# arnavdantuluri/StableTriton

Hardware: AMD Instinct MI355X
Metric: denoise it/s, SDXL UNet 1024x1024 50-step, bs=1 per GPU (higher is better)
Workload: dtype bf16; 1 GPU; SDXL-base UNet, latent 128x128 (1024x1024 px), bs=1/GPU, 50-step Euler-discrete loop, hipGraph mode=step, no CFG; parallelism=prompt-parallel x1, weights=synthetic seed 0, weight_broadcasts=0

## Files before the change

### stabletriton_amd/csrc/conv_thin.h

```cpp
#pragma once
#include "gemm_args.h"

template <typename T, int KMAX>
__global__ __launch_bounds__(256) void conv_thin_kernel(const GemmArgs p, int R, int chunk) {
    extern __shared__ __attribute__((aligned(16))) float wsm[];
    const T* x = (const T*)p.A;
    const T* w = (const T*)p.W;
    const int K = p.K, N = p.N;
    const int n_lo = blockIdx.y * chunk, n_hi = min(N, n_lo + chunk);
    for (int i = threadIdx.x; i < K * (n_hi - n_lo); i += 256) {
        const int nl = i / K, k = i - nl * K;
        wsm[k * chunk + nl] = Elem<T>::to_f(w[(size_t)(n_lo + nl) * K + k]);
    }
    __syncthreads();
    const int m = blockIdx.x * 256 + threadIdx.x;
    const bool live = m < p.M;
    const int mm = live ? m : 0;
    const int hw = p.Hout * p.Wout;
    const int img = mm / hw, rem = mm - img * hw;
    const int oy = rem / p.Wout, ox = rem - oy * p.Wout;
    float xin[KMAX];
#pragma unroll
    for (int k = 0; k < KMAX; ++k) xin[k] = 0.f;
    if (R == 3 && p.S == 3 && p.Cin == 4 && KMAX >= 36) {
#pragma unroll
        for (int r = 0; r < 3; ++r)
#pragma unroll
            for (int s_ = 0; s_ < 3; ++s_) {
                int iy = oy * p.stride - p.pad + r, ix = ox * p.stride - p.pad + s_;
                const int He = p.ups ? 2 * p.Hin : p.Hin, We = p.ups ? 2 * p.Win : p.Win;
                const bool ok = iy >= 0 && ix >= 0 && iy < He && ix < We;
                if (p.ups) { iy >>= 1; ix >>= 1; }
                const T* xp = x + (((size_t)img * p.Hin + (ok ? iy : 0)) * p.Win + (ok ? ix : 0)) * 4;
                float f[4];
                Out4<T>::load(xp, f);
#pragma unroll
                for (int c = 0; c < 4; ++c) xin[(r * 3 + s_) * 4 + c] = ok ? f[c] : 0.f;
            }
    } else {
        int k = 0;
        for (int r = 0; r < R; ++r)
            for (int s_ = 0; s_ < p.S; ++s_) {
                int iy = oy * p.stride - p.pad + r, ix = ox * p.stride - p.pad + s_;
                const int He = p.ups ? 2 * p.Hin : p.Hin, We = p.ups ? 2 * p.Win : p.Win;
                const bool ok = iy >= 0 && ix >= 0 && iy < He && ix < We;
                if (p.ups) { iy >>= 1; ix >>= 1; }
                const T* xp = x + (((size_t)img * p.Hin + (ok ? iy : 0)) * p.Win + (ok ? ix : 0)) * p.Cin;
                for (int c = 0; c < p.Cin; ++c, ++k) {
                    const float v = ok ? Elem<T>::to_f(xp[c]) : 0.f;
#pragma unroll
                    for (int kk = 0; kk < KMAX; ++kk) if (kk == k) xin[kk] = v;
                }
            }
    }
    for (int n0 = n_lo; n0 < n_hi; n0 += 16) {
        float acc[16];
#pragma unroll
        for (int e = 0; e < 16; ++e) acc[e] = 0.f;
#pragma unroll
        for (int k = 0; k < KMAX; ++k) {
            if (k < K) {
                const float xv = xin[k];
                const float* wr = wsm + k * chunk + (n0 - n_lo);
#pragma unroll
                for (int e = 0; e < 16; e += 4) {
                    const f32x4 w4 = *reinterpret_cast<const f32x4*>(wr + e);
                    acc[e] += xv * w4[0]; acc[e + 1] += xv * w4[1]; acc[e + 2] += xv * w4[2]; acc[e + 3] += xv * w4[3];
                }
            }
        }
        if (!live) continue;
#pragma unroll
        for (int e0 = 0; e0 < 16; e0 += 4) {
            const int co = n0 + e0;
            if (co >= N) break;
            float v[4] = {acc[e0], acc[e0 + 1], acc[e0 + 2], acc[e0 + 3]};
            if (p.epi & ST_EPI_BIAS)
                for (int e = 0; e < 4; ++e) v[e] += Elem<T>::to_f(((const T*)p.bias)[co + e]);
            if (p.epi & ST_EPI_SILU)
                for (int e = 0; e < 4; ++e) v[e] = silu_f(v[e]);
            if (p.epi & ST_EPI_ROWBIAS)
                for (int e = 0; e < 4; ++e) v[e] += Elem<T>::to_f(((const T*)p.rowbias)[(size_t)(m / p.rows_per_batch) * N + co + e]);
            if (p.epi & ST_EPI_RESIDUAL)
                for (int e = 0; e < 4; ++e) v[e] += Elem<T>::to_f(((const T*)p.residual)[(size_t)m * p.ldr + co + e]);
            Out4<T>::store((T*)p.C + (size_t)m * p.ldc + co, v);
        }
    }
}

template <typename T>
static int conv_thin_launch(const GemmArgs& a, int R, hipStream_t st) {
    const int bx = cdiv(a.M, 256);
    int ny = cdiv(1024, bx);
    if (ny > a.N / 16) ny = a.N / 16;
    if (ny < 1) ny = 1;
    const int chunk = cdiv(cdiv(a.N, ny), 16) * 16;
    ny = cdiv(a.N, chunk);
    const size_t lds = (size_t)a.K * chunk * sizeof(float);
    ST_REQUIRE(lds <= 64 * 1024, "conv2d(thin): weights do not fit LDS");
    hipLaunchKernelGGL((conv_thin_kernel<T, 64>), dim3(bx, ny), dim3(256), lds, st, a, R, chunk);
    return st_check_launch("conv2d(thin)");
}
```

### stabletriton_amd/csrc/dispatch.h

```cpp
#pragma once
#include "gemm_reg.h"
#include "gemm_dma.h"
#include "gemm8p.h"
#ifdef ST_DEV_CONFIGS
#include "../../tools/dev_kernels/gemm4w.h"
void gemm4w_bf16(const GemmArgs& a, hipStream_t st);
void gemm4w_f16(const GemmArgs& a, hipStream_t st);
void gemm4w_fp8(const GemmArgs& a, hipStream_t st);
template <typename T> static inline void gemm4w_call(const GemmArgs& a, hipStream_t st) {
    if constexpr (std::is_same<T, bf16>::value) gemm4w_bf16(a, st);
    else if constexpr (std::is_same<T, f16>::value) gemm4w_f16(a, st);
    else gemm4w_fp8(a, st);
}
#endif

static inline bool colstats_ok(const GemmArgs& a, int bm, bool lnf) {
    const bool ok = a.col_stats && !lnf && (a.N & 3) == 0 && a.rows_per_batch > 0 && a.rows_per_batch % bm == 0 &&
                    cdiv(a.M, bm) <= a.col_tiles_cap;
    if (a.col_rows_out) *a.col_rows_out = ok ? bm : 0;
    return ok;
}

template <typename T, int BM, int BN, int WGM, int WGN, int STAGES, int U, bool CONV, bool GEGLU, bool LNF, bool XA = false>
static void launch_dma_one(const GemmArgs& a, hipStream_t st, int tiles_n) {
    const size_t lds = (size_t)STAGES * U * (BM + BN) * 128 + (size_t)BM * 8 + 1024;
    const int sk = a.splitk > 1 ? a.splitk : 1;
    auto kfn = gemm_dma_kernel<T, BM, BN, WGM, WGN, STAGES, U, CONV, GEGLU, LNF, XA>;
    const bool emit_cols = colstats_ok(a, BM, LNF);
    static unsigned long long lds_ok = 0;
    ensure_dynamic_lds(kfn, lds, &lds_ok);
    GemmArgs b = a;
    {
        static const int force_pm = dev_env_int("ST_GEMM_PANELS", 0);
        const int tiles_m = cdiv(a.M, BM);
        const double abytes = CONV ? (double)a.M * a.Cin * (a.ups ? 0.25 : 1.0) * a.stride * a.stride : (double)a.M * a.K;
        const double wbytes = (double)(GEGLU ? 2 : 1) * a.N * a.K;
        int best_p = 1;
        double best = 1e300;
        for (int pm = 1; pm <= 8; pm *= 2) {
            if (pm > tiles_m) break;
            const double c = abytes * (8.0 / pm) + wbytes * pm;
            if (c < best) { best = c; best_p = pm; }
        }
        if (force_pm > 0) best_p = force_pm > tiles_m ? tiles_m : force_pm;
        b.panel_h = cdiv(tiles_m, best_p);
    }
    const int main_blocks = cdiv(a.M, BM) * tiles_n * sk;
    b.splitk = sk;
    fill_tile_map(b, cdiv(a.M, BM), tiles_n, a.K / ((128 / (int)sizeof(T)) * U));
    static const bool no_helpers = dev_env_int("ST_NO_HELPER_BLOCKS", 0) != 0;
    b.helper_blocks = (b.next_w && main_blocks <= 208 && !no_helpers) ? (256 - main_blocks > 96 ? 96 : 256 - main_blocks) : 0;
    if (!emit_cols) b.col_stats = nullptr;
    fill_next_per(b, main_blocks + b.helper_blocks);
    hipLaunchKernelGGL(kfn, dim3(main_blocks + b.helper_blocks), dim3(WGM * WGN * 64), lds, st, b);
}

template <typename T, int BM, int BN, int WGM, int WGN, int STAGES, int U, bool CONV>
static void launch_dma(const GemmArgs& a, hipStream_t st) {
    if constexpr (!CONV) {
        const bool geglu = a.epi & ST_EPI_GEGLU;
        constexpr bool PAIRS = (BN % 32 == 0);
        if (a.ln_c) {
            if constexpr (PAIRS) {
                if (geglu) { launch_dma_one<T, BM, BN, WGM, WGN, STAGES, U, false, true, true>(a, st, cdiv(a.N, BN / 2)); return; }
            }
            launch_dma_one<T, BM, BN, WGM, WGN, STAGES, U, false, false, true>(a, st, cdiv(a.N, BN));
            return;
        }
        if constexpr (PAIRS) {
            if (geglu) { launch_dma_one<T, BM, BN, WGM, WGN, STAGES, U, false, true, false>(a, st, cdiv(a.N, BN / 2)); return; }
        }
    }
    launch_dma_one<T, BM, BN, WGM, WGN, STAGES, U, CONV, false, false>(a, st, cdiv(a.N, BN));
}

enum { CFG_64x64_S4 = 0, CFG_64x64_S8 = 1, CFG_64x64_S4_U2 = 2, CFG_128x64_S4 = 3, CFG_128x64_S3_U2 = 4,
       CFG_128x128_S3 = 5, CFG_64x64_S3 = 6, CFG_64x64_W8 = 7, CFG_128x64_W8 = 8, CFG_128x128_W8 = 9,
       CFG_64x128_W8 = 10, CFG_64x128_W8_S6 = 11, CFG_128x64_W8_S6 = 12, CFG_128x128_W8_S4 = 13, CFG_64x64_W8_S8 = 14, CFG_64x128_W8_U2 = 15, CFG_128x64_W8_U2 = 16, CFG_64x64_W8_U2 = 17, CFG_256x256_W8 = 18, CFG_256x128_W8 = 19, CFG_128x128_W8_S2 = 20, CFG_128x64_W8_S3 = 21, CFG_64x128_W8_S3 = 22, CFG_128x320_W8 = 23, CFG_128x256_W8 = 24, CFG_64x320_W8 = 25, CFG_64x80_W4 = 26, CFG_128x80_W8 = 27, CFG_128x160_W8 = 28, CFG_128x128_N4_S2 = 29, CFG_128x64_N4_S3 = 30, CFG_64x128_N4_S3 = 31, CFG_256x160_W8_S2 = 32, CFG_COUNT, CFG_256x256_8P = 100, CFG_256x160_8P = 101, CFG_256x256_4W = 102 };

static inline int cfg_bn(int cfg) {
    switch (cfg) {
        case CFG_64x64_S4: case CFG_64x64_S8: case CFG_64x64_S4_U2: case CFG_128x64_S4: case CFG_128x64_S3_U2: case CFG_64x64_S3:
        case CFG_64x64_W8: case CFG_128x64_W8: case CFG_128x64_W8_S6: case CFG_64x64_W8_S8: case CFG_128x64_W8_U2:
        case CFG_64x64_W8_U2: case CFG_128x64_W8_S3: case CFG_128x64_N4_S3: return 64;
        case CFG_256x256_W8: case CFG_128x256_W8: return 256;
        case CFG_128x320_W8: case CFG_64x320_W8: return 320;
        case CFG_64x80_W4: case CFG_128x80_W8: return 80;
        case CFG_128x160_W8: case CFG_256x160_W8_S2: return 160;
        default: return 128;
    }
}

#ifdef ST_DEV_CONFIGS
extern int g_dbg_cfg, g_dbg_fusek;
#endif
static inline int forced_cfg() {
    static int v = dev_env_int("ST_GEMM_FORCE", -1);
#ifdef ST_DEV_CONFIGS
    if (g_dbg_cfg >= 0) return g_dbg_cfg;
#endif
    return v;
}

#ifndef ST_TW_128x128
#define ST_TW_128x128 1.0
#endif
#ifndef ST_TW_64x128
#define ST_TW_64x128 1.0
#endif
#ifndef ST_TW_128x64
#define ST_TW_128x64 1.0
#endif
#ifndef ST_TW_64x64
#define ST_TW_64x64 1.0
#endif
#ifndef ST_TW_128x80
#define ST_TW_128x80 1.0
#endif
#ifndef ST_TW_128x160
#define ST_TW_128x160 1.0
#endif
#ifndef ST_TW_SPLITK
#define ST_TW_SPLITK 1.0
#endif
#ifndef ST_TW_8P
#define ST_TW_8P 1.1
#endif
static inline double model_tweak(int cfg) {
    switch (cfg) {
        case 9: return ST_TW_128x128;
        case 10: return ST_TW_64x128;
        case 8: return ST_TW_128x64;
        case 7: return ST_TW_64x64;
        case 27: return ST_TW_128x80;
        case 28: return ST_TW_128x160;
        default: return 1.0;
    }
}
#ifndef ST_SPLIT_DENSE_TRIP
#define ST_SPLIT_DENSE_TRIP 1.0
#endif
#ifndef ST_SPLIT_160_TRIP
#define ST_SPLIT_160_TRIP 0.8
#endif
template <typename T, bool CONV>
static int gemm_dispatch(const GemmArgs& a_in, hipStream_t st, int depth = 0) {
    GemmArgs a = a_in;
    if (a.Ng == 0) a.Ng = a.N;
    const long n_eff = (a.epi & ST_EPI_GEGLU) ? 2L * a.N : a.N;
    auto tiles = [&](int bm, int bn) { return (long)cdiv(a.M, bm) * cdiv(n_eff, bn); };
    constexpr int KB = 128 / (int)sizeof(T);
    const char* who = CONV ? "conv2d" : "linear";
    if constexpr (frag2<T>()) {
        if (a.K % KB != 0) return st_fail("%s: fp8 / split fp32 operands need K to be a multiple of %d", who, KB);
    } else if (a.K % KB != 0) {
        if (a.stats_chunks_out) *a.stats_chunks_out = 0;
        if (tiles(128, 128) >= 240) launch_cfg<T, 128, 128, 2, 2, CONV>(a, st);
        else if (tiles(128, 64) >= 200) launch_cfg<T, 128, 64, 2, 2, CONV>(a, st);
        else launch_cfg<T, 64, 64, 2, 2, CONV>(a, st);
        return st_check_launch(who);
    }
    if constexpr (std::is_same<T, float>::value) {
        GemmArgs b = a;
        b.stats_chunks = cdiv(a.N, 64);
        if (a.stats_chunks_out) *a.stats_chunks_out = a.row_stats ? b.stats_chunks : 0;
        launch_dma<T, 64, 64, 2, 2, 4, 1, CONV>(b, st);
        return st_check_launch(who);
    } else {
        const bool even2 = (a.K % (2 * KB) == 0);
        struct Cand { int cfg, bm, bn; double trip_us; };
        static const Cand cands[] = {{CFG_128x128_W8, 128, 128, 0.53}, {CFG_64x128_W8, 64, 128, 0.34}, {CFG_128x64_W8, 128, 64, 0.32},
                                     {CFG_64x64_W8, 64, 64, 0.19}, {CFG_128x320_W8, 128, 320, 1.9}, {CFG_64x320_W8, 64, 320, 1.1},
                                     {CFG_256x128_W8, 256, 128, 0.72}, {CFG_128x80_W8, 128, 80, 0.37}, {CFG_128x160_W8, 128, 160, 0.66}};
        static const int sks[] = {1, 2, 3, 4, 6, 8};
        static const int force_sk = dev_env_int("ST_GEMM_SPLITK", -1);
        const int nk = a.K / KB;
        const long ncols = (a.epi & ST_EPI_GEGLU) ? 2L * a.N : a.N;
        const bool can_split = a.partial && !a.ln_c && force_sk != 0 && force_sk != 1;
        int cfg = CFG_64x64_W8, sk = 1;
        double best = 1e30;
        auto small_model = [&](long ncols_, int* cfg_out, int* sk_out) {
            auto tiles_ = [&](int bm, int bn) { return (long)cdiv(a.M, bm) * cdiv(ncols_, bn); };
            double best_ = 1e30;
            for (const Cand& c : cands) {
                if (frag2<T>() && c.bn == 320) continue;
                if (is_split<T>() && c.cfg == CFG_256x128_W8) continue;
                if ((a.epi & ST_EPI_GEGLU) && c.bn % 32 != 0) continue;
                const long nt = tiles_(c.bm, c.bn);
                const double trip = (is_split<T>() && c.cfg == CFG_128x160_W8 ? ST_SPLIT_160_TRIP : c.trip_us * (is_split<T>() && !CONV ? ST_SPLIT_DENSE_TRIP : 1.0)) * (CONV ? 1.6 : 1.0) * ((!CONV && sizeof(T) == 2) ? model_tweak(c.cfg) : 1.0);
                for (int k_ : sks) {
                    if (k_ > 1 && (!can_split || nk / k_ < 4 || nt > 16384)) break;
                    const double slab_mb = (double)k_ * nt * c.bm * c.bn * 4.0 / 1e6;
                    if (k_ > 1 && slab_mb * 1e6 + 65536 > (double)a.partial_bytes) break;
                    const double rounds = (double)((nt * k_ + 255) / 256);
                    const double in_round = (double)(nt * k_ < 256 ? nt * k_ : 256);
                    const double trip_bw = in_round * (c.bm + c.bn) * 128.0 / 14.0e6;
                    const double cost = rounds * (cdiv(nk, k_) * (trip > trip_bw ? trip : trip_bw) + 3.0) * (rounds > 1.0 ? 1.3 : 1.0) + (k_ > 1 ? (2.1 + 0.4 * slab_mb) * ((!CONV && sizeof(T) == 2) ? ST_TW_SPLITK : 1.0) : 0.0);
                    if (cost < best_) { best_ = cost; if (cfg_out) *cfg_out = c.cfg; if (sk_out) *sk_out = k_; }
                }
            }
            return best_;
        };
        best = small_model(ncols, &cfg, &sk);
        if constexpr (!CONV && sizeof(T) <= 2) {
            const int f = forced_cfg();
            double c256 = 1e30, c160 = 1e30;
            if (gemm8p_applies(a, 256, KB)) c256 = (double)((tiles(256, 256) + 255) / 256) * (nk * 1.65 + 4.0);
            if (gemm8p_applies(a, 160, KB)) c160 = (double)((tiles(256, 160) + 255) / 256) * (nk * 1.52 + 4.0);
#ifdef ST_DEV_CONFIGS
            if (f == CFG_256x256_4W && gemm4w_applies(a, KB)) { gemm4w_call<T>(a, st); return st_check_launch(who); }
#endif
            static const bool no_colsplit = dev_env_int("ST_NO_COLSPLIT", 0) != 0;
            if (f < 0 && depth == 0 && !no_colsplit && c256 < 1e29 && !a.row_stats && !a.col_stats && !a.q8_out && !a.sp_out && !a.row_scale) {
                const long tm = a.M / 256, total = tiles(256, 256);
                const long rem = total % 256;
                if (total > 256 && rem > 0 && rem <= 128 && 256 % tm == 0) {
                    const long full_cols = (total / 256) * (256 / tm);
                    const long rem_rows = n_eff - full_cols * 256;
                    const double c_full = (double)(total / 256) * (nk * 1.65 + 4.0);
                    const double c_split = c_full + small_model(rem_rows, nullptr, nullptr) + 2.5;
                    const double c_whole = c256 < c160 ? c256 : c160;
                    if (c_split < 0.93 * (c_whole < best ? c_whole : best)) {
                        const int bno = (a.epi & ST_EPI_GEGLU) ? 128 : 256;
                        const long n1 = full_cols * bno;
                        typedef typename OutT<T>::type TO_;
                        GemmArgs a1 = a, a2 = a;
                        a1.N = (int)n1;
                        a1.next_w = (const char*)a.W + (size_t)n1 * a.K * sizeof(T); a1.next_bytes = (size_t)(a.N - n1) * a.K * sizeof(T); a1.next_row_lines = 0; a1.next_lead_shift = 0;
                        a2.N = a.N - (int)n1;
                        a2.W = (const char*)a.W + (size_t)n1 * a.K * sizeof(T);
                        a2.C = (char*)a.C + (size_t)n1 * sizeof(TO_);
                        if (a.bias) a2.bias = (const char*)a.bias + (size_t)n1 * sizeof(TO_);
                        if (a.residual) a2.residual = (const char*)a.residual + (size_t)n1 * sizeof(TO_);
                        if (a.ln_c) { a2.ln_c = a.ln_c + n1; a2.ln_d = a.ln_d + n1; }
                        if (a.col_scale) a2.col_scale = a.col_scale + n1;
                        if (a.stats_chunks_out) *a.stats_chunks_out = 0;
                        gemm8p_launch<T, 256, 2, 4>(a1, st);
                        if (int e = st_check_launch(who)) return e;
                        return gemm_dispatch<T, CONV>(a2, st, depth + 1);
                    }
                }
            }
            const bool take256 = f == CFG_256x256_8P || (f < 0 && c256 <= c160 && c256 < ST_TW_8P * best);
            const bool take160 = f == CFG_256x160_8P || (f < 0 && c160 < c256 && c160 < ST_TW_8P * best);
            if (take256 && c256 < 1e29) { gemm8p_launch<T, 256, 2, 4>(a, st); return st_check_launch(who); }
            if (take160 && c160 < 1e29) { gemm8p_launch<T, 160, 4, 2>(a, st); return st_check_launch(who); }
        }
        if constexpr (!CONV && is_split<T>()) {
            const int f = forced_cfg();
            double c160 = 1e30;
            if (gemm8p_applies(a, 160, KB)) c160 = (double)((tiles(256, 160) + 255) / 256) * (nk * 1.15 + 5.0);
            if (c160 < 1e29 && (f == CFG_256x160_8P || (f < 0 && c160 < 0.9 * best))) { gemm8p_launch<T, 160, 4, 2>(a, st); return st_check_launch(who); }
        }
        GemmArgs b = a;
#ifdef ST_DEV_CONFIGS
        {
            static const int small_cfg = dev_env_int("ST_GEMM_SMALL_CFG", -1);
            if (small_cfg >= 0 && small_cfg < CFG_COUNT && tiles(128, 128) < 150 && sk == 1) cfg = small_cfg;
        }
#endif
        {
            static const int env_fk = dev_env_int("ST_GEMM_FUSEK", -1);
            int force_fk = env_fk;
#ifdef ST_DEV_CONFIGS
            if (g_dbg_cfg >= 0) force_fk = g_dbg_fusek;
#endif
            const int f = forced_cfg();
            if (f >= 0 && f < CFG_COUNT) {
                const bool u2 = (f == CFG_64x64_S4_U2 || f == CFG_128x64_S3_U2 || f == CFG_64x128_W8_U2 || f == CFG_128x64_W8_U2 ||
                                 f == CFG_64x64_W8_U2);
                if (!u2 || even2) { cfg = f; sk = (force_fk > 1 && can_split) ? (force_fk > nk ? nk : force_fk) : 1; }
            }
        }
        if (sk > 1) {
            int bm = 128;
            if (cfg == CFG_64x64_W8 || cfg == CFG_64x128_W8 || cfg == CFG_64x320_W8 || cfg == CFG_64x80_W4) bm = 64;
            if (cfg == CFG_256x128_W8 || cfg == CFG_256x160_W8_S2) bm = 256;
            const long nt = tiles(bm, cfg_bn(cfg));
            if (nt <= 16384 && (size_t)sk * nt * bm * cfg_bn(cfg) * 4 + 65536 <= a.partial_bytes) {
                b.splitk = sk; b.tile_counters = (int*)a.partial; b.partial = a.partial + 16384;
            }
        }
        b.stats_chunks = cdiv(a.N, cfg_bn(cfg));
        if (a.row_stats && b.stats_chunks > a.stats_capacity) return st_fail("%s: row_stats buffer holds %d chunks, %d needed", who, a.stats_capacity, b.stats_chunks);
        if (a.stats_chunks_out) *a.stats_chunks_out = a.row_stats ? b.stats_chunks : 0;
        switch (cfg) {
            case CFG_64x64_W8: launch_dma<T, 64, 64, 4, 2, 4, 1, CONV>(b, st); break;
            case CFG_128x64_W8: launch_dma<T, 128, 64, 4, 2, 4, 1, CONV>(b, st); break;
            case CFG_64x128_W8: launch_dma<T, 64, 128, 2, 4, 4, 1, CONV>(b, st); break;
            case CFG_256x128_W8: launch_dma<T, 256, 128, 4, 2, 3, 1, CONV>(b, st); break;
            case CFG_128x320_W8: launch_dma<T, 128, 320, 4, 2, 2, 1, CONV>(b, st); break;
            case CFG_64x320_W8: launch_dma<T, 64, 320, 2, 4, 3, 1, CONV>(b, st); break;
            case CFG_128x80_W8: launch_dma<T, 128, 80, 8, 1, 4, 1, CONV>(b, st); break;
            case CFG_128x160_W8:
                if constexpr (is_split<T>()) launch_dma<T, 128, 160, 4, 2, 4, 1, CONV>(b, st);
                else launch_dma<T, 128, 160, 8, 1, 4, 1, CONV>(b, st);
                break;
#ifdef ST_DEV_CONFIGS
            case CFG_64x80_W4: launch_dma<T, 64, 80, 4, 1, 6, 1, CONV>(b, st); break;
            case CFG_128x256_W8: launch_dma<T, 128, 256, 4, 2, 3, 1, CONV>(b, st); break;
            case CFG_64x64_S4: launch_dma<T, 64, 64, 2, 2, 4, 1, CONV>(b, st); break;
            case CFG_64x64_S8: launch_dma<T, 64, 64, 2, 2, 8, 1, CONV>(b, st); break;
            case CFG_64x64_S4_U2: launch_dma<T, 64, 64, 2, 2, 4, 2, CONV>(b, st); break;
            case CFG_128x64_S4: launch_dma<T, 128, 64, 2, 2, 4, 1, CONV>(b, st); break;
            case CFG_128x64_S3_U2: launch_dma<T, 128, 64, 2, 2, 3, 2, CONV>(b, st); break;
            case CFG_128x128_S3: launch_dma<T, 128, 128, 2, 2, 3, 1, CONV>(b, st); break;
            case CFG_64x64_S3: launch_dma<T, 64, 64, 2, 2, 3, 1, CONV>(b, st); break;
            case CFG_128x128_N4_S2: launch_dma<T, 128, 128, 2, 2, 2, 1, CONV>(b, st); break;
            case CFG_128x64_N4_S3: launch_dma<T, 128, 64, 2, 2, 3, 1, CONV>(b, st); break;
            case CFG_64x128_N4_S3: launch_dma<T, 64, 128, 2, 2, 3, 1, CONV>(b, st); break;
            case CFG_256x160_W8_S2: launch_dma<T, 256, 160, 4, 2, 2, 1, CONV>(b, st); break;
            case CFG_64x128_W8_S6: launch_dma<T, 64, 128, 2, 4, 6, 1, CONV>(b, st); break;
            case CFG_128x64_W8_S6: launch_dma<T, 128, 64, 4, 2, 6, 1, CONV>(b, st); break;
            case CFG_128x128_W8_S4: launch_dma<T, 128, 128, 2, 4, 3, 1, CONV>(b, st); break;
            case CFG_64x64_W8_S8: launch_dma<T, 64, 64, 4, 2, 8, 1, CONV>(b, st); break;
            case CFG_64x128_W8_U2: launch_dma<T, 64, 128, 2, 4, 3, 2, CONV>(b, st); break;
            case CFG_128x64_W8_U2: launch_dma<T, 128, 64, 4, 2, 3, 2, CONV>(b, st); break;
            case CFG_64x64_W8_U2: launch_dma<T, 64, 64, 4, 2, 4, 2, CONV>(b, st); break;
            case CFG_256x256_W8: launch_dma<T, 256, 256, 2, 4, 2, 1, CONV>(b, st); break;
            case CFG_128x128_W8_S2: launch_dma<T, 128, 128, 2, 4, 2, 1, CONV>(b, st); break;
            case CFG_128x64_W8_S3: launch_dma<T, 128, 64, 4, 2, 3, 1, CONV>(b, st); break;
            case CFG_64x128_W8_S3: launch_dma<T, 64, 128, 2, 4, 3, 1, CONV>(b, st); break;
#endif
            default: launch_dma<T, 128, 128, 2, 4, 4, 1, CONV>(b, st); break;
        }
        return st_check_launch(who);
    }
}


static inline void take_hint(GemmArgs& a, const void* next_w, size_t next_bytes) {
    const size_t row_lines = (next_bytes >> 40) & 0xfffff, shift = (next_bytes >> 60) & 3;
    next_bytes &= ((size_t)1 << 40) - 1;
    a.next_row_lines = 0; a.next_lead_shift = 0;
    if (next_w && row_lines && (row_lines >> shift) >= 2 && next_bytes >= (row_lines << 7)) {
        const size_t rows = (next_bytes >> 7) / row_lines;
        a.next_row_lines = (unsigned)row_lines; a.next_lead_shift = (unsigned)shift;
        next_bytes = (rows << shift) << 7;
    }
    a.next_w = next_bytes ? next_w : nullptr;
    a.next_bytes = next_w ? next_bytes : 0;
}

static inline int check_epilogue(const char* who, const GemmArgs& a) {
    ST_REQUIRE(!(a.epi & ST_EPI_BIAS) || a.bias, "%s: ST_EPI_BIAS without bias pointer", who);
    ST_REQUIRE(!(a.epi & ST_EPI_RESIDUAL) || a.residual, "%s: ST_EPI_RESIDUAL without residual pointer", who);
    ST_REQUIRE(!(a.epi & ST_EPI_ROWBIAS) || (a.rowbias && a.rows_per_batch > 0), "%s: ST_EPI_ROWBIAS needs rowbias and rows_per_batch", who);
    ST_REQUIRE(!((a.epi & ST_EPI_GEGLU) && (a.epi & ST_EPI_SILU)), "%s: GEGLU and SILU are exclusive", who);
    return 0;
}
```

### stabletriton_amd/csrc/gemm8p.h

```cpp
#pragma once
#include "gemm_dma.h"

template <int BN, int WGM, int WGN> constexpr bool TILE_OK_SPLIT() { return (256 / WGM / 16) * (BN / WGN / 16) <= 20; }
template <typename T, bool GEGLU, bool LNF, int BN = 256, int WGM = 2, int WGN = 4, bool DIRECT = false>
__global__ __launch_bounds__(512) void gemm8p_kernel(const GemmArgs p) {
    static_assert(sizeof(T) <= 2 || is_split<T>(), "16-bit elements (bf16 / f16), e4m3 bytes, or split fp32 operands (strict mode: 256 x 160 tiles)");
    static_assert(!is_split<T>() || (TILE_OK_SPLIT<BN, WGM, WGN>()), "split operands carry two accumulator sets: wave tiles of at most 64 x 80");
    constexpr int BM = 256, NW = 8;
    constexpr int KB = 128 / (int)sizeof(T);
    constexpr int EV = 16 / (int)sizeof(T);
    typedef typename OutT<T>::type TO;
    static_assert(WGM * WGN == NW && BM % (32 * WGM) == 0 && BN % (16 * WGN) == 0 && (!GEGLU || BN % 32 == 0), "wave layout");
    constexpr int WTM = BM / WGM, WTN = BN / WGN, TM = WTM / 16, TN = WTN / 16;
    constexpr int TMH = TM / 2, TN0 = (TN + 1) / 2, TN1 = TN - TN0;
    constexpr int RA = WGM * TMH * 16, RB0 = WGN * TN0 * 16, RB1 = WGN * TN1 * 16;
    static_assert(RA == 128 && RB0 <= 128 && RB1 <= 128 && RB0 % 8 == 0 && RB1 % 8 == 0, "a region is at most sixteen 8-row pieces");
    constexpr int HA = RA * 128, HB0 = RB0 * 128, HB1 = RB1 * 128;
    constexpr int TILE_B = 2 * HA + HB0 + HB1;
    constexpr int BNO = GEGLU ? BN / 2 : BN;
    typedef typename Mma<T>::Frag Frag;
    typedef typename std::conditional<frag2<T>(), u32x4, Frag>::type Half;
    extern __shared__ __attribute__((aligned(16))) char lds[];
    char* const lnrows = lds + 2 * TILE_B;
    char* const dump = lnrows + BM * 8;

    const int t = threadIdx.x, lane = t & 63;
    const int wave = __builtin_amdgcn_readfirstlane(t >> 6);
    const int wm = wave / WGN, wn = wave - wm * WGN;
    const int tiles_m = p.M / BM;
    const int nblk = gridDim.x - p.helper_blocks, bid = blockIdx.x;
    if (bid >= nblk) {
        unsigned int sink = 0;
        touch_next_weights(p, sink, true);
        retire_touches(sink);
        return;
    }
    const TileId tid = tile_of_block(p, bid, nblk);
    const int tile_m = tid.tile_m, tile_n = tid.tile_n;
    const int m0 = tile_m * BM, n0 = tile_n * BNO;
#ifdef ST_PROBE8
    unsigned long long pr_t0 = __builtin_readcyclecounter(), pr_t1 = 0, pr_t2 = 0, pr_r0 = __builtin_amdgcn_s_memrealtime();
#endif
    const T* __restrict__ Ap = (const T*)p.A;
    const T* __restrict__ Wp = (const T*)p.W;
    const T* zeros = reinterpret_cast<const T*>(g_zero16);

    const int lr = lane >> 3;
    const int lc = (lane & 7) ^ lr;
    const T* a_src[2];
    const T* b0_src[2];
    const T* b1_src[2];
    auto w_row = [&](int c) { return GEGLU ? (c < BN / 2 ? (size_t)(n0 + c) : (size_t)p.Ng + n0 + (c - BN / 2)) : (size_t)(n0 + c); };
    auto w_row_direct = [&](int wc, int j, int rho) {
        const DirectCol dc = direct_col<TN, GEGLU>(j, rho);
        return (size_t)(dc.gate ? p.Ng : 0) + n0 + wc * (GEGLU ? WTN / 2 : WTN) + dc.col;
    };
#pragma unroll
    for (int e = 0; e < 2; ++e) {
        const int idx = (2 * wave + e) * 8 + lr;
        a_src[e] = Ap + (size_t)(m0 + (idx / (TMH * 16)) * WTM + (idx % (TMH * 16))) * p.lda + lc * EV;
        const int i0 = idx < RB0 ? idx : 0, i1 = idx < RB1 ? idx : 0;
        if constexpr (DIRECT) {
            const int in0 = i0 % (TN0 * 16), in1 = i1 % (TN1 * 16);
            b0_src[e] = Wp + w_row_direct(i0 / (TN0 * 16), in0 >> 4, in0 & 15) * p.K + lc * EV;
            b1_src[e] = Wp + w_row_direct(i1 / (TN1 * 16), TN0 + (in1 >> 4), in1 & 15) * p.K + lc * EV;
        } else {
            b0_src[e] = Wp + w_row((i0 / (TN0 * 16)) * WTN + (i0 % (TN0 * 16))) * p.K + lc * EV;
            b1_src[e] = Wp + w_row((i1 / (TN1 * 16)) * WTN + TN0 * 16 + (i1 % (TN1 * 16))) * p.K + lc * EV;
        }
    }
    const size_t a_half = (size_t)(TMH * 16) * p.lda;
    const int nk = p.K / KB;

    auto issue_half = [&](int kt, int region) {
#ifdef ST_PROBE8
        if (p.korder & 2) kt = nk;
#endif
        const int roff = region == 0 ? 0 : region == 1 ? HA : region == 2 ? 2 * HA : 2 * HA + HB0;
        const int rrows = region < 2 ? RA : region == 2 ? RB0 : RB1;
        const unsigned dst = lds_addr_of(lds) + (kt & 1) * TILE_B + roff + (2 * wave) * 1024;
#pragma unroll
        for (int e = 0; e < 2; ++e) {
            const bool live = kt < nk && (2 * wave + e) * 8 < rrows;
            const T* src = region < 2 ? a_src[e] + (region & 1) * a_half : region == 2 ? b0_src[e] : b1_src[e];
            src = live ? src + (size_t)kt * KB : zeros;
            dma16_at<0>(src, live ? dst + e * 1024 : lds_addr_of(lds) + 2 * TILE_B + BM * 8);
        }
    };

    unsigned int touch_sink = 0;
    {
        auto touch_at = [&](const char* a) {
            a = (const char*)((uintptr_t)a & ~(uintptr_t)3);
            asm volatile("global_load_dword %0, %1, off" : "+v"(touch_sink) : "v"(a) : "memory");
        };
        auto touch = [&](const void* base, long byte_off, int nbytes) {
            for (int o = t * 128; o < nbytes; o += 512 * 128) touch_at((const char*)base + byte_off + o);
        };
        if (p.epi & ST_EPI_BIAS) {
            touch(p.bias, (long)n0 * (long)sizeof(TO), BNO * (int)sizeof(TO));
            if (GEGLU) touch(p.bias, ((long)p.Ng + n0) * (long)sizeof(TO), BNO * (int)sizeof(TO));
        }
        if (LNF) {
            touch(p.ln_c, (long)n0 * 4, BNO * 4); touch(p.ln_d, (long)n0 * 4, BNO * 4);
            if (GEGLU) { touch(p.ln_c, ((long)p.Ng + n0) * 4, BNO * 4); touch(p.ln_d, ((long)p.Ng + n0) * 4, BNO * 4); }
        }
        if (p.epi & ST_EPI_RESIDUAL) {
            constexpr int lines = (BNO * (int)sizeof(TO) + 127) / 128;
            for (int o = t; o < BM * lines; o += 512) {
                const int r = o / lines, l = o - r * lines;
                touch_at((const char*)p.residual + ((size_t)(m0 + r) * p.ldr + n0) * sizeof(TO) + l * 128);
            }
        }
    }
    LnRowSum<2> ln_sum;
    if constexpr (LNF) {
        const float2* st2 = reinterpret_cast<const float2*>(p.ln_stats);
        const int row = t >> 1, part = t & 1;
        ln_sum.load(st2 + (size_t)(m0 + row) * p.ln_chunks, p.ln_chunks, part);
    }
    issue_half(0, 0); issue_half(0, 2); issue_half(0, 3); issue_half(0, 1); issue_half(1, 0); issue_half(1, 2); issue_half(1, 3);
    if constexpr (LNF) {
        const float2* st2 = reinterpret_cast<const float2*>(p.ln_stats);
        const int row = t >> 1, part = t & 1;
        float a1, a2;
        ln_sum.finish(st2 + (size_t)(m0 + row) * p.ln_chunks, p.ln_chunks, part, a1, a2);
        const float mean = a1 / (float)p.K;
        const float rstd = rsqrtf(fmaxf(a2 / (float)p.K - mean * mean, 0.f) + p.ln_eps);
        if (part == 0) reinterpret_cast<float2*>(lnrows)[row] = make_float2(mean, rstd);
        asm volatile("s_waitcnt lgkmcnt(0)" ::: "memory");
    }
    wait_vmcnt<8>();
    __builtin_amdgcn_s_barrier();
    asm volatile("" ::"v"(touch_sink));
    if (wave >= 4) __builtin_amdgcn_s_barrier();

    f32x4 acc[TM][TN];
    f32x4 corr[is_split<T>() ? TM : 1][is_split<T>() ? TN : 1];
#pragma unroll
    for (int i = 0; i < TM; ++i)
#pragma unroll
        for (int j = 0; j < TN; ++j) {
            acc[i][j] = (f32x4){0.f, 0.f, 0.f, 0.f};
            if constexpr (is_split<T>()) corr[i][j] = (f32x4){0.f, 0.f, 0.f, 0.f};
        }

    const int r16 = lane & 15, q = lane >> 4;
    int a_off[2], b0_off[2], b1_off[2];
#pragma unroll
    for (int kk = 0; kk < 2; ++kk) {
        const int sw = ((4 * kk + q) ^ (r16 & 7)) << 4;
        a_off[kk] = (wm * TMH * 16 + r16) * 128 + sw;
        b0_off[kk] = 2 * HA + (wn * TN0 * 16 + r16) * 128 + sw;
        b1_off[kk] = 2 * HA + HB0 + (wn * TN1 * 16 + r16) * 128 + sw;
    }
    constexpr int NKK = frag2<T>() ? 1 : 2;
    Frag fa[TMH][NKK], fb[TN][NKK];
    auto read_op = [&](const char* base, const int (&off)[2], Frag (&dst)[NKK]) {
        if constexpr (frag2<T>()) {
            const Half lo = *reinterpret_cast<const Half*>(base + off[0]), hi = *reinterpret_cast<const Half*>(base + off[1]);
            dst[0] = Frag{(int)lo[0], (int)lo[1], (int)lo[2], (int)lo[3], (int)hi[0], (int)hi[1], (int)hi[2], (int)hi[3]};
        } else {
#pragma unroll
            for (int kk = 0; kk < 2; ++kk) dst[kk] = *reinterpret_cast<const Frag*>(base + off[kk]);
        }
    };
    auto read_a = [&](const char* tile, int h) {
#pragma unroll
        for (int i = 0; i < TMH; ++i) read_op(tile + h * HA + i * 2048, a_off, fa[i]);
    };
    auto read_b = [&](const char* tile) {
#pragma unroll
        for (int j = 0; j < TN0; ++j) read_op(tile + j * 2048, b0_off, fb[j]);
#pragma unroll
        for (int j = 0; j < TN1; ++j) read_op(tile + j * 2048, b1_off, fb[TN0 + j]);
    };
    auto half_tile = [&](auto mh_) {
        constexpr int mh = decltype(mh_)::value;
#ifdef ST_PROBE8
        if (p.korder & 1) return;
#endif
        __builtin_amdgcn_s_setprio(1);
#pragma unroll
        for (int kk = 0; kk < NKK; ++kk)
#pragma unroll
            for (int i = 0; i < TMH; ++i)
#pragma unroll
                for (int j = 0; j < TN; ++j) {
                    if constexpr (is_split<T>()) Mma<T>::run2(acc[mh * TMH + i][j], corr[mh * TMH + i][j], fb[j][kk], fa[i][kk]);
                    else Mma<T>::run(acc[mh * TMH + i][j], fb[j][kk], fa[i][kk]);
                }
        __builtin_amdgcn_s_setprio(0);
    };
#define ST_PHASE_SYNC()                                   \
    __builtin_amdgcn_sched_barrier(0);                    \
    wait_vmcnt<8>();                                      \
    __builtin_amdgcn_s_barrier();                         \
    __builtin_amdgcn_sched_barrier(0)
#define ST_PHASE_END()                                    \
    __builtin_amdgcn_sched_barrier(0);                    \
    __builtin_amdgcn_s_barrier();                         \
    __builtin_amdgcn_sched_barrier(0)
    typedef std::integral_constant<int, 0> I0;
    typedef std::integral_constant<int, 1> I1;
#ifdef ST_PROBE8
    pr_t1 = __builtin_readcyclecounter();
#endif
    for (int kt = 0; kt < nk; ++kt) {
        const char* tile = lds + (kt & 1) * TILE_B;
        read_a(tile, 0); read_b(tile);
        issue_half(kt + 1, 1);
        ST_PHASE_SYNC();
        half_tile(I0{});
        ST_PHASE_END();
        read_a(tile, 1);
        issue_half(kt + 2, 0); issue_half(kt + 2, 2); issue_half(kt + 2, 3);
        ST_PHASE_SYNC();
        half_tile(I1{});
        ST_PHASE_END();
    }
#undef ST_PHASE_SYNC
#undef ST_PHASE_END
    if (wave < 4) __builtin_amdgcn_s_barrier();
    wait_vmcnt<0>();
    __builtin_amdgcn_s_barrier();
#ifdef ST_PROBE8
    pr_t2 = __builtin_readcyclecounter();
#endif
    if constexpr (is_split<T>()) {
#pragma unroll
        for (int i = 0; i < TM; ++i)
#pragma unroll
            for (int j = 0; j < TN; ++j)
#pragma unroll
                for (int e = 0; e < 4; ++e) acc[i][j][e] = __builtin_fmaf(corr[i][j][e], ST_SPLIT_INV, acc[i][j][e]);
    }
    if constexpr (DIRECT)
        direct_epilogue<TO, TM, TN, WTM, WTN, WGM, WGN, GEGLU, LNF>(p, acc, m0, n0, tile_n, wm, wn, r16, q, lds, reinterpret_cast<const float2*>(lnrows),
                                                                    lds_addr_of(lds) + 2 * TILE_B + BM * 8);
    else
        staged_epilogue<TO, BM, BN, WGM, WGN, TM, TN, GEGLU, 2 * TILE_B, !LNF, is_fp8<T>()>(p, acc, m0, n0, tile_n, wm, r16, q, ColsPlain{wn, WTN}, lds,
                                                                            reinterpret_cast<const float2*>(lnrows));
#ifdef ST_PROBE8
    asm volatile("s_waitcnt vmcnt(0)" ::: "memory");
    if (p.partial && t == 0) {
        unsigned long long* o = reinterpret_cast<unsigned long long*>(reinterpret_cast<char*>(p.partial) + 65536) + (size_t)bid * 8;
        o[0] = pr_t0; o[1] = pr_t1; o[2] = pr_t2; o[3] = __builtin_readcyclecounter(); o[4] = pr_r0; o[5] = __builtin_amdgcn_s_memrealtime();
    }
#endif
}

static inline bool gemm8p_applies(const GemmArgs& a, int bn, int kb = 64) {
    const long n_rows = (a.epi & ST_EPI_GEGLU) ? 2L * a.N : a.N;
    return a.M % 256 == 0 && n_rows % bn == 0 && a.K % kb == 0 && a.K >= 2 * kb && a.N % 8 == 0 &&
           !(a.epi & ST_EPI_ROWBIAS) && (!a.row_stats || !(a.epi & ST_EPI_GEGLU));
}

template <typename T, bool GEGLU, bool LNF, int BN, int WGM, int WGN, bool DIRECT = false>
static void gemm8p_go(const GemmArgs& a, hipStream_t st) {
    constexpr size_t lds = 2 * (size_t)(2 * 128 * 128 + BN * 128) + 256 * 8 + 1024;
    auto kfn = gemm8p_kernel<T, GEGLU, LNF, BN, WGM, WGN, DIRECT>;
    static unsigned long long lds_ok = 0;
    ensure_dynamic_lds(kfn, lds, &lds_ok);
    GemmArgs b = a;
    const int tiles_m = a.M / 256, tiles_n = (int)(((a.epi & ST_EPI_GEGLU) ? 2L * a.N : a.N) / BN);
    {
        const double abytes = (double)a.M * a.K, wbytes = (double)tiles_n * BN * a.K;
        int best_p = 1;
        double best = 1e300;
        for (int pm = 1; pm <= 8 && pm <= tiles_m; pm *= 2) {
            const double c = abytes * (8.0 / pm) + wbytes * pm;
            if (c < best) { best = c; best_p = pm; }
        }
        b.panel_h = cdiv(tiles_m, best_p);
    }
    const int main_blocks = tiles_m * tiles_n;
    b.splitk = 1;
    fill_tile_map(b, tiles_m, tiles_n, 0);
    b.helper_blocks = (b.next_w && main_blocks <= 208) ? (256 - main_blocks > 96 ? 96 : 256 - main_blocks) : 0;
    b.stats_chunks = tiles_n;
    if (a.stats_chunks_out) *a.stats_chunks_out = a.row_stats ? b.stats_chunks : 0;
    if (!colstats_ok(a, 256, LNF)) b.col_stats = nullptr;
    fill_next_per(b, main_blocks + b.helper_blocks);
    hipLaunchKernelGGL(kfn, dim3(main_blocks + b.helper_blocks), dim3(512), lds, st, b);
}

template <typename T>
static inline bool gemm8p_direct(const GemmArgs& a, bool tall) {
    if constexpr (sizeof(T) != 2) return false;
    static const bool off = dev_env_int("ST_8P_STAGED", 0) != 0;
    if (off || direct_flags(a, a.ln_c != nullptr, tall) < 0) return false;
    auto al16 = [](const void* p_) { return ((uintptr_t)p_ & 15) == 0; };
    return a.ldc % 8 == 0 && al16(a.C) && (!(a.epi & ST_EPI_RESIDUAL) || (a.ldr % 8 == 0 && al16(a.residual))) && al16(a.bias) && al16(a.ln_c) && al16(a.ln_d);
}

template <typename T, int BN, int WGM, int WGN>
static void gemm8p_launch(const GemmArgs& a, hipStream_t st) {
    const bool geglu = a.epi & ST_EPI_GEGLU;
    if constexpr (sizeof(T) == 2) {
        if (gemm8p_direct<T>(a, 256 / WGM / 16 >= 8)) {
            if (a.ln_c) { if (geglu) gemm8p_go<T, true, true, BN, WGM, WGN, true>(a, st); else gemm8p_go<T, false, true, BN, WGM, WGN, true>(a, st); }
            else { if (geglu) gemm8p_go<T, true, false, BN, WGM, WGN, true>(a, st); else gemm8p_go<T, false, false, BN, WGM, WGN, true>(a, st); }
            return;
        }
    }
    if (a.ln_c) { if (geglu) gemm8p_go<T, true, true, BN, WGM, WGN>(a, st); else gemm8p_go<T, false, true, BN, WGM, WGN>(a, st); }
    else { if (geglu) gemm8p_go<T, true, false, BN, WGM, WGN>(a, st); else gemm8p_go<T, false, false, BN, WGM, WGN>(a, st); }
}
```

### stabletriton_amd/csrc/gemm_api.hip

```cpp
#include "gemm_core.h"

#ifdef ST_DEV_CONFIGS
int g_dbg_cfg = -1, g_dbg_fusek = -1;
extern "C" void st_debug_force_gemm(int cfg, int fusek) { g_dbg_cfg = cfg; g_dbg_fusek = fusek; }
#endif

static int run_dense(const GemmArgs& a, int dtype, hipStream_t st) {
    switch (dtype) {
        case ST_BF16: return gemm_dense_bf16(a, st);
        case ST_F16: return gemm_dense_f16(a, st);
        case ST_F32S: return gemm_dense_f32s(a, st);
        default: return gemm_dense_f32(a, st);
    }
}

static int check_q8(const char* who, GemmArgs& a, void* q8, long ldq8, const float* q8_inv_scale, unsigned int* q8_amax) {
    if (!q8) return 0;
    ST_REQUIRE(q8_inv_scale && q8_amax, "%s: the e4m3 copy needs its scale and its amax slots", who);
    ST_REQUIRE(a.N % 8 == 0 && ldq8 % 8 == 0 && (uintptr_t)q8 % 8 == 0, "%s: e4m3 copy: N and its row stride must be multiples of 8", who);
    a.q8_out = q8; a.q8_ld = ldq8; a.q8_inv_scale = q8_inv_scale; a.q8_amax = q8_amax;
    return 0;
}

static int linear_impl(const void* x, const void* W, const void* bias, const void* residual, const void* rowbias, void* y,
                       int M, int N, int K, long lda, long ldc, long ldr, int rows_per_batch, int epilogue, int dtype,
                       void* workspace, size_t workspace_bytes, float* row_stats, int row_stats_capacity,
                       int* row_stats_chunks, float* col_stats, int col_stats_tiles, int* col_stats_rows,
                       void* q8, long ldq8, const float* q8_inv_scale, unsigned int* q8_amax,
                       const void* next_weights, size_t next_weights_bytes, void* stream) {
    if (col_stats_rows) *col_stats_rows = 0;
    ST_REQUIRE(x && W && y, "linear: null pointer");
    ST_REQUIRE(M > 0 && N > 0 && K > 0, "linear: bad shape M=%d N=%d K=%d", M, N, K);
    ST_REQUIRE(st_dtype_ok_gemm(dtype), "linear: unsupported dtype %d", dtype);
    const int vec = st_dtype_is16(dtype) ? 8 : (dtype == ST_F32S ? 32 : 4);
    ST_REQUIRE(K % vec == 0 && lda % vec == 0, "linear: K=%d and lda=%ld must be multiples of %d", K, lda, vec);
    ST_REQUIRE(ldc % 4 == 0 && (!(epilogue & ST_EPI_RESIDUAL) || ldr % 4 == 0), "linear: ldc/ldr must be multiples of 4");
    ST_REQUIRE(((uintptr_t)x | (uintptr_t)W) % 16 == 0 && (uintptr_t)y % 16 == 0, "linear: pointers must be 16-byte aligned");
    GemmArgs a = {};
    a.A = x; a.W = W; a.bias = bias; a.residual = residual; a.rowbias = rowbias; a.C = y;
    a.M = M; a.N = N; a.K = K; a.lda = lda; a.ldc = ldc; a.ldr = ldr; a.rows_per_batch = rows_per_batch; a.epi = epilogue;
    a.splitk = 1; a.partial = (float*)workspace; a.partial_bytes = workspace ? workspace_bytes : 0;
    ST_REQUIRE(!row_stats || !(epilogue & ST_EPI_GEGLU), "linear: row_stats with GEGLU is not supported");
    a.row_stats = row_stats; a.stats_capacity = row_stats_capacity; a.stats_chunks_out = row_stats_chunks;
    a.col_stats = col_stats; a.col_tiles_cap = col_stats_tiles; a.col_rows_out = col_stats_rows;
    take_hint(a, next_weights, next_weights_bytes);
#ifdef ST_PROBE8
    { const char* e_ = getenv("ST_PROBE_KNOB"); a.korder = e_ ? atoi(e_) : 0; }
#endif
    if (int e = check_epilogue("linear", a)) return e;
    if (q8) {
        ST_REQUIRE(st_dtype_is16(dtype), "linear: the e4m3 copy is emitted by the 16-bit kernels");
        if (int e = check_q8("linear", a, q8, ldq8, q8_inv_scale, q8_amax)) return e;
    }
    if (int e = st_take_split_arm("linear", M, N, !st_dtype_is16(dtype) && N % 32 == 0, &a.sp_out)) return e;
    return run_dense(a, dtype, (hipStream_t)stream);
}

extern "C" int st_linear(const void* x, const void* W, const void* bias, const void* residual, const void* rowbias, void* y,
                         int M, int N, int K, long lda, long ldc, long ldr, int rows_per_batch, int epilogue, int dtype,
                         void* workspace, size_t workspace_bytes, float* row_stats, int row_stats_capacity,
                         int* row_stats_chunks, float* col_stats, int col_stats_tiles, int* col_stats_rows,
                         const void* next_weights, size_t next_weights_bytes, void* stream) {
    return linear_impl(x, W, bias, residual, rowbias, y, M, N, K, lda, ldc, ldr, rows_per_batch, epilogue, dtype, workspace, workspace_bytes,
                       row_stats, row_stats_capacity, row_stats_chunks, col_stats, col_stats_tiles, col_stats_rows, nullptr, 0, nullptr, nullptr,
                       next_weights, next_weights_bytes, stream);
}

extern "C" int st_linear_emit8(const void* x, const void* W, const void* bias, const void* residual, const void* rowbias, void* y,
                               int M, int N, int K, long lda, long ldc, long ldr, int rows_per_batch, int epilogue, int dtype,
                               void* workspace, size_t workspace_bytes, float* row_stats, int row_stats_capacity,
                               int* row_stats_chunks, float* col_stats, int col_stats_tiles, int* col_stats_rows,
                               void* q8, long ldq8, const float* q8_inv_scale, unsigned int* q8_amax,
                               const void* next_weights, size_t next_weights_bytes, void* stream) {
    ST_REQUIRE(q8, "linear_emit8: null e4m3 output");
    return linear_impl(x, W, bias, residual, rowbias, y, M, N, K, lda, ldc, ldr, rows_per_batch, epilogue, dtype, workspace, workspace_bytes,
                       row_stats, row_stats_capacity, row_stats_chunks, col_stats, col_stats_tiles, col_stats_rows, q8, ldq8, q8_inv_scale, q8_amax,
                       next_weights, next_weights_bytes, stream);
}

extern "C" int st_ln_linear(const void* x, const float* row_stats, int row_stats_chunks, const void* Wg, const float* c,
                            const float* d, void* y, int M, int N, int K, long lda, long ldc, float eps, int epilogue,
                            int dtype, const void* next_weights, size_t next_weights_bytes, void* stream) {
    ST_REQUIRE(x && Wg && c && d && y && row_stats, "ln_linear: null pointer");
    ST_REQUIRE(row_stats_chunks > 0, "ln_linear: the producer emitted no row statistics");
    ST_REQUIRE(M > 0 && N > 0 && K > 0, "ln_linear: bad shape M=%d N=%d K=%d", M, N, K);
    ST_REQUIRE(st_dtype_ok_gemm(dtype), "ln_linear: unsupported dtype %d", dtype);
    const int kb = st_dtype_is16(dtype) ? 64 : 32;
    ST_REQUIRE(K % kb == 0 && lda % (dtype == ST_F32S ? 32 : kb / 8) == 0, "ln_linear: K=%d must be a multiple of %d", K, kb);
    ST_REQUIRE(ldc % 4 == 0, "ln_linear: ldc must be a multiple of 4");
    ST_REQUIRE((epilogue & ~ST_EPI_GEGLU) == 0, "ln_linear: only the GEGLU epilogue flag is accepted (bias lives in d)");
    ST_REQUIRE(((uintptr_t)x | (uintptr_t)Wg | (uintptr_t)y) % 16 == 0, "ln_linear: pointers must be 16-byte aligned");
    GemmArgs a = {};
    a.A = x; a.W = Wg; a.C = y; a.M = M; a.N = N; a.K = K; a.lda = lda; a.ldc = ldc; a.epi = epilogue;
    a.ln_c = c; a.ln_d = d; a.ln_eps = eps; a.splitk = 1; a.ln_stats = row_stats; a.ln_chunks = row_stats_chunks;
    take_hint(a, next_weights, next_weights_bytes);
    if (int e = st_take_split_arm("ln_linear", M, N, !st_dtype_is16(dtype) && N % 32 == 0, &a.sp_out)) return e;
    return run_dense(a, dtype, (hipStream_t)stream);
}

extern "C" int st_ln_linear_xattn(const void* x, const float* row_stats, int row_stats_chunks, const void* Wg, const float* c,
                                  const float* d, const void* k, const void* v, void* out, int M, int N, int K, long lda, long ldo,
                                  float eps, int rows_per_batch, int S, int H, long ldk, long ldv, float scale, int dtype,
                                  const void* next_weights, size_t next_weights_bytes, void* stream) {
    ST_REQUIRE(st_dtype_is16(dtype), "ln_linear_xattn: dtype %d not supported (bf16 / f16)", dtype);
    ST_REQUIRE(x && Wg && c && d && k && v && out && row_stats, "ln_linear_xattn: null pointer");
    ST_REQUIRE(row_stats_chunks > 0, "ln_linear_xattn: the producer emitted no row statistics");
    ST_REQUIRE(M > 0 && N > 0 && K > 0 && S > 0 && H > 0, "ln_linear_xattn: bad shape M=%d N=%d K=%d S=%d H=%d", M, N, K, S, H);
    ST_REQUIRE(N == H * 64, "ln_linear_xattn: N=%d must be H*64 (H=%d)", N, H);
    ST_REQUIRE(S < 256, "ln_linear_xattn: context of %d keys (the fused epilogue runs the short-context attention core: S < 256)", S);
    ST_REQUIRE(rows_per_batch > 0 && rows_per_batch % 128 == 0 && M % rows_per_batch == 0,
               "ln_linear_xattn: %d rows per batch: query tiles of 128 rows must not straddle batches", rows_per_batch);
    ST_REQUIRE(K % 64 == 0 && lda % 8 == 0 && ldo % 4 == 0 && ldk % 8 == 0 && ldv % 8 == 0, "ln_linear_xattn: K, strides must keep 16-byte alignment");
    ST_REQUIRE(((uintptr_t)x | (uintptr_t)Wg | (uintptr_t)out | (uintptr_t)k | (uintptr_t)v | (uintptr_t)c | (uintptr_t)d) % 16 == 0,
               "ln_linear_xattn: pointers must be 16-byte aligned");
    GemmArgs a = {};
    a.A = x; a.W = Wg; a.C = out; a.M = M; a.N = N; a.K = K; a.lda = lda; a.ldc = ldo; a.epi = 0;
    a.ln_c = c; a.ln_d = d; a.ln_eps = eps; a.splitk = 1; a.ln_stats = row_stats; a.ln_chunks = row_stats_chunks;
    a.xa_k = k; a.xa_v = v; a.xa_ldk = ldk; a.xa_ldv = ldv; a.xa_S = S; a.xa_T = rows_per_batch; a.xa_scale_log2e = scale * 1.4426950408889634f;
    take_hint(a, next_weights, next_weights_bytes);
    { void* none; if (int e = st_take_split_arm("ln_linear_xattn", M, N, false, &none)) return e; }
    return dtype == ST_BF16 ? gemm_xattn_bf16(a, (hipStream_t)stream) : gemm_xattn_f16(a, (hipStream_t)stream);
}

extern "C" int st_linear_fp8(const void* xq, const float* row_scale, const void* Wq, const float* w_scale, const void* bias,
                             const void* residual, void* y, int M, int N, int K, long lda, long ldc, long ldr, int epilogue,
                             void* workspace, size_t workspace_bytes, const void* next_weights, size_t next_weights_bytes,
                             void* stream) {
    ST_REQUIRE(xq && row_scale && Wq && w_scale && y, "linear_fp8: null pointer");
    ST_REQUIRE(M > 0 && N > 0 && K > 0, "linear_fp8: bad shape M=%d N=%d K=%d", M, N, K);
    ST_REQUIRE(K % 128 == 0 && lda % 16 == 0, "linear_fp8: K=%d must be a multiple of 128 and lda=%ld of 16", K, lda);
    ST_REQUIRE(N % 4 == 0 && ldc % 4 == 0 && (!(epilogue & ST_EPI_RESIDUAL) || ldr % 4 == 0), "linear_fp8: N, ldc, ldr must be multiples of 4");
    ST_REQUIRE(!(epilogue & ST_EPI_ROWBIAS), "linear_fp8: the row-bias epilogue is not supported");
    ST_REQUIRE(((uintptr_t)xq | (uintptr_t)Wq | (uintptr_t)y | (uintptr_t)w_scale) % 16 == 0, "linear_fp8: pointers must be 16-byte aligned");
    GemmArgs a = {};
    a.A = xq; a.W = Wq; a.bias = bias; a.residual = residual; a.C = y;
    a.M = M; a.N = N; a.K = K; a.lda = lda; a.ldc = ldc; a.ldr = ldr; a.epi = epilogue;
    a.row_scale = row_scale; a.col_scale = w_scale; a.rs_stride = 1;
    a.splitk = 1; a.partial = (float*)workspace; a.partial_bytes = workspace ? workspace_bytes : 0;
    take_hint(a, next_weights, next_weights_bytes);
    if (int e = check_epilogue("linear_fp8", a)) return e;
    return gemm_dense_fp8(a, (hipStream_t)stream);
}

extern "C" int st_linear_fp8x(const void* xq, const float* a_scale, int a_scale_stride, const void* Wq, const float* w_scale,
                              const void* bias, const void* residual, void* y, int M, int N, int K, long lda, long ldc, long ldr, int epilogue,
                              const float* ln_stats, int ln_chunks, const float* ln_c, const float* ln_d, float ln_eps,
                              float* row_stats, int row_stats_capacity, int* row_stats_chunks,
                              void* q8, long ldq8, const float* q8_inv_scale, unsigned int* q8_amax,
                              void* workspace, size_t workspace_bytes, const void* next_weights, size_t next_weights_bytes, void* stream) {
    ST_REQUIRE(xq && a_scale && Wq && w_scale && (y || q8), "linear_fp8x: null pointer");
    ST_REQUIRE(a_scale_stride == 0 || a_scale_stride == 1, "linear_fp8x: activation scale stride %d (0 = per tensor, 1 = per row)", a_scale_stride);
    ST_REQUIRE(M > 0 && N > 0 && K > 0, "linear_fp8x: bad shape M=%d N=%d K=%d", M, N, K);
    ST_REQUIRE(K % 128 == 0 && lda % 16 == 0, "linear_fp8x: K=%d must be a multiple of 128 and lda=%ld of 16", K, lda);
    ST_REQUIRE(N % 4 == 0 && (!y || ldc % 4 == 0) && (!(epilogue & ST_EPI_RESIDUAL) || ldr % 4 == 0), "linear_fp8x: N, ldc, ldr must be multiples of 4");
    ST_REQUIRE(!(epilogue & ST_EPI_ROWBIAS), "linear_fp8x: the row-bias epilogue is not supported");
    ST_REQUIRE(((uintptr_t)xq | (uintptr_t)Wq | (uintptr_t)y | (uintptr_t)w_scale) % 16 == 0, "linear_fp8x: pointers must be 16-byte aligned");
    ST_REQUIRE(!ln_c || (ln_d && ln_stats && ln_chunks > 0 && !(epilogue & ~ST_EPI_GEGLU)), "linear_fp8x: folded LayerNorm takes c, d, the row statistics and only the GEGLU flag (bias lives in d)");
    ST_REQUIRE(y || (epilogue & ST_EPI_GEGLU), "linear_fp8x: an output without y (only the e4m3 copy) is the GEGLU form");
    GemmArgs a = {};
    a.A = xq; a.W = Wq; a.bias = bias; a.residual = residual; a.C = y;
    a.M = M; a.N = N; a.K = K; a.lda = lda; a.ldc = ldc; a.ldr = ldr; a.epi = epilogue;
    a.row_scale = a_scale; a.col_scale = w_scale; a.rs_stride = a_scale_stride;
    a.ln_c = ln_c; a.ln_d = ln_d; a.ln_eps = ln_eps; a.ln_stats = ln_stats; a.ln_chunks = ln_chunks;
    a.splitk = 1; a.partial = (float*)workspace; a.partial_bytes = workspace ? workspace_bytes : 0;
    ST_REQUIRE(!row_stats || !(epilogue & ST_EPI_GEGLU), "linear_fp8x: row_stats with GEGLU is not supported");
    a.row_stats = row_stats; a.stats_capacity = row_stats_capacity; a.stats_chunks_out = row_stats_chunks;
    take_hint(a, next_weights, next_weights_bytes);
    if (int e = check_epilogue("linear_fp8x", a)) return e;
    if (int e = check_q8("linear_fp8x", a, q8, ldq8, q8_inv_scale, q8_amax)) return e;
    return gemm_dense_fp8(a, (hipStream_t)stream);
}

extern "C" int st_conv2d(const void* x, const void* W, const void* bias, const void* residual, const void* rowbias, void* y,
                         int N, int Hin, int Win, int Cin, int Cout, int R, int S, int stride, int pad, int upsample2x,
                         int epilogue, int dtype, void* workspace, size_t workspace_bytes,
                         float* col_stats, int col_stats_tiles, int* col_stats_rows,
                         const void* next_weights, size_t next_weights_bytes, void* stream) {
    if (col_stats_rows) *col_stats_rows = 0;
    ST_REQUIRE(x && W && y, "conv2d: null pointer");
    ST_REQUIRE(N > 0 && Hin > 0 && Win > 0 && Cin > 0 && Cout > 0 && R > 0 && S > 0 && stride > 0 && pad >= 0,
               "conv2d: bad geometry");
    ST_REQUIRE(st_dtype_ok_gemm(dtype), "conv2d: unsupported dtype %d", dtype);
    ST_REQUIRE(!(epilogue & ST_EPI_GEGLU), "conv2d: GEGLU epilogue not supported");
    ST_REQUIRE(Cout % 4 == 0, "conv2d: Cout=%d must be a multiple of 4", Cout);
    const int He = upsample2x ? 2 * Hin : Hin, We = upsample2x ? 2 * Win : Win;
    GemmArgs a = {};
    a.A = x; a.W = W; a.bias = bias; a.residual = residual; a.rowbias = rowbias; a.C = y;
    a.Hin = Hin; a.Win = Win; a.Cin = Cin; a.S = S; a.stride = stride; a.pad = pad; a.ups = upsample2x ? 1 : 0;
    {
        static const int korder_env = dev_env_int("ST_CONV_KORDER", -1);
        a.R_ = R; a.korder = korder_env >= 0 ? korder_env : 0;
    }
    a.Hout = (He + 2 * pad - R) / stride + 1;
    a.Wout = (We + 2 * pad - S) / stride + 1;
    ST_REQUIRE(a.Hout > 0 && a.Wout > 0, "conv2d: empty output");
    a.M = N * a.Hout * a.Wout; a.N = Cout; a.K = R * S * Cin;
    a.lda = 0; a.ldc = Cout; a.ldr = Cout; a.rows_per_batch = a.Hout * a.Wout; a.epi = epilogue;
    a.splitk = 1; a.partial = (float*)workspace; a.partial_bytes = workspace ? workspace_bytes : 0;
    a.col_stats = col_stats; a.col_tiles_cap = col_stats_tiles; a.col_rows_out = col_stats_rows;
    take_hint(a, next_weights, next_weights_bytes);
    if (int e = check_epilogue("conv2d", a)) return e;
    if (int e = st_take_split_arm("conv2d", a.M, Cout, !st_dtype_is16(dtype) && Cout % 32 == 0 && Cin % 32 == 0, &a.sp_out)) return e;
    hipStream_t st = (hipStream_t)stream;
    const int kb = st_dtype_is16(dtype) ? 64 : 32;
    if (Cin % kb == 0) {
        ST_REQUIRE(((uintptr_t)x | (uintptr_t)W | (uintptr_t)y) % 16 == 0, "conv2d: pointers must be 16-byte aligned");
        if (dtype == ST_BF16) return gemm_conv_bf16(a, R, upsample2x, st);
        if (dtype == ST_F16) return gemm_conv_f16(a, R, upsample2x, st);
        if (dtype == ST_F32S) return gemm_conv_f32s(a, R, upsample2x, st);
        return gemm_conv_f32(a, st);
    }
    ST_REQUIRE(dtype != ST_F32S, "conv2d: split fp32 operands need Cin=%d to be a multiple of 32 (thin inputs take plain ST_F32)", Cin);
    ST_REQUIRE(a.K <= 64 && Cout % 16 == 0, "conv2d: Cin=%d is neither a multiple of %d (implicit GEMM) nor thin (R*S*Cin <= 64, Cout %% 16 == 0)", Cin, kb);
    return conv_thin_run(a, R, dtype, st);
}

extern "C" int st_conv1x1_cat(const void* x0, int C0, const void* x1, int C1, const void* W, const void* bias, const void* residual, void* y,
                              int N, int H, int Wd, int Cout, int epilogue, int dtype, void* workspace, size_t workspace_bytes,
                              float* col_stats, int col_stats_tiles, int* col_stats_rows,
                              const void* next_weights, size_t next_weights_bytes, void* stream) {
    if (col_stats_rows) *col_stats_rows = 0;
    ST_REQUIRE(x0 && x1 && W && y, "conv1x1_cat: null pointer");
    ST_REQUIRE(N > 0 && H > 0 && Wd > 0 && C0 > 0 && C1 > 0 && Cout > 0, "conv1x1_cat: bad geometry");
    ST_REQUIRE(st_dtype_ok_gemm(dtype), "conv1x1_cat: unsupported dtype %d", dtype);
    ST_REQUIRE(!(epilogue & (ST_EPI_GEGLU | ST_EPI_ROWBIAS)), "conv1x1_cat: GEGLU / row-bias epilogues not supported");
    ST_REQUIRE(Cout % 4 == 0, "conv1x1_cat: Cout=%d must be a multiple of 4", Cout);
    const int kb = st_dtype_is16(dtype) ? 64 : 32;
    ST_REQUIRE(C0 % kb == 0 && C1 % kb == 0, "conv1x1_cat: both channel counts (%d, %d) must be multiples of %d", C0, C1, kb);
    ST_REQUIRE(((uintptr_t)x0 | (uintptr_t)x1 | (uintptr_t)W | (uintptr_t)y) % 16 == 0, "conv1x1_cat: pointers must be 16-byte aligned");
    GemmArgs a = {};
    a.A = x0; a.A2 = x1; a.Csplit = C0; a.W = W; a.bias = bias; a.residual = residual; a.C = y;
    a.Hin = H; a.Win = Wd; a.Cin = C0 + C1; a.S = 1; a.stride = 1; a.pad = 0; a.ups = 0; a.R_ = 1; a.korder = 0;
    a.Hout = H; a.Wout = Wd;
    a.M = N * H * Wd; a.N = Cout; a.K = C0 + C1;
    a.lda = 0; a.ldc = Cout; a.ldr = Cout; a.rows_per_batch = H * Wd; a.epi = epilogue;
    a.splitk = 1; a.partial = (float*)workspace; a.partial_bytes = workspace ? workspace_bytes : 0;
    a.col_stats = col_stats; a.col_tiles_cap = col_stats_tiles; a.col_rows_out = col_stats_rows;
    take_hint(a, next_weights, next_weights_bytes);
    if (int e = check_epilogue("conv1x1_cat", a)) return e;
    if (int e = st_take_split_arm("conv1x1_cat", a.M, Cout, !st_dtype_is16(dtype) && Cout % 32 == 0, &a.sp_out)) return e;
    hipStream_t st = (hipStream_t)stream;
    if (dtype == ST_BF16) return gemm_conv_bf16(a, 1, 0, st);
    if (dtype == ST_F16) return gemm_conv_f16(a, 1, 0, st);
    if (dtype == ST_F32S) return gemm_conv_f32s(a, 1, 0, st);
    return gemm_conv_f32(a, st);
}
```

### stabletriton_amd/csrc/gemm_args.h

```cpp
#pragma once
#include "common.h"
#include "attention_core.h"
#include "split.h"
#include <stdlib.h>
#include <type_traits>

struct GemmArgs {
    const void* A; const void* W; const void* bias; const void* residual; const void* rowbias; void* C;
    int M, N, K;
    int Ng;
    long lda, ldc, ldr;
    int rows_per_batch;
    int epi;
    int Hin, Win, Cin, Hout, Wout, S, stride, pad, ups;
    int R_, korder;
    const float* ln_c; const float* ln_d; float ln_eps;
    const float* ln_stats; int ln_chunks;
    float* row_stats; int stats_chunks;
    int stats_capacity; int* stats_chunks_out;
    float* col_stats; int col_tiles_cap; int* col_rows_out;
    int splitk;
    float* partial;
    size_t partial_bytes;
    int* tile_counters;
    int panel_h;
    const void* A2; int Csplit;
    int tm_tiles_m, tm_per_panel, tm_last_rows, tm_slow;
    unsigned tm_mg_splitk, tm_mg_per_panel, tm_mg_rows, tm_mg_last;
    int nk_base, nk_rem;
    unsigned next_per;
    unsigned next_row_lines;
    unsigned next_lead_shift;
    const float* row_scale; const float* col_scale;
    int rs_stride;
    void* q8_out; long q8_ld; const float* q8_inv_scale; unsigned int* q8_amax;
    void* sp_out;
    const void* next_w; size_t next_bytes;
    int helper_blocks;
    const void* xa_k; const void* xa_v; long xa_ldk, xa_ldv; int xa_S, xa_T; float xa_scale_log2e;
};

static inline int dev_env_int(const char* name, int dflt) {
#ifdef ST_DEV_CONFIGS
    const char* e = getenv(name);
    return e ? atoi(e) : dflt;
#else
    (void)name;
    return dflt;
#endif
}

static inline bool colstats_ok(const GemmArgs& a, int bm, bool lnf);

template <typename T> struct Mma;
template <> struct Mma<bf16> {
    typedef bf16x8 Frag;
    static __device__ __forceinline__ void run(f32x4& acc, const Frag& a, const Frag& b) {
        acc = __builtin_amdgcn_mfma_f32_16x16x32_bf16(a, b, acc, 0, 0, 0);
    }
};
template <> struct Mma<f16> {
    typedef f16x8 Frag;
    static __device__ __forceinline__ void run(f32x4& acc, const Frag& a, const Frag& b) {
        acc = __builtin_amdgcn_mfma_f32_16x16x32_f16(a, b, acc, 0, 0, 0);
    }
};
template <> struct Mma<float> {
    typedef f32x4 Frag;
    static __device__ __forceinline__ void run(f32x4& acc, const Frag& a, const Frag& b) {
#pragma unroll
        for (int j = 0; j < 4; ++j) acc = __builtin_amdgcn_mfma_f32_16x16x4f32(a[j], b[j], acc, 0, 0, 0);
    }
};

struct f8 { unsigned char v; };
typedef __attribute__((ext_vector_type(8))) int i32x8;
template <> struct Mma<f8> {
    typedef i32x8 Frag;
    static __device__ __forceinline__ void run(f32x4& acc, const Frag& a, const Frag& b) {
        acc = __builtin_amdgcn_mfma_scale_f32_16x16x128_f8f6f4(a, b, acc, 0 , 0 , 0, 0x7F7F7F7F, 0, 0x7F7F7F7F);
    }
};
struct fsp { float raw; };
template <> struct Mma<fsp> {
    typedef i32x8 Frag;
    static __device__ __forceinline__ void run2(f32x4& acc, f32x4& corr, const Frag& a, const Frag& b) {
        typedef __attribute__((ext_vector_type(4))) int i32x4_;
        const f16x8 ah = __builtin_bit_cast(f16x8, (i32x4_)__builtin_shufflevector(a, a, 0, 1, 2, 3));
        const f16x8 al = __builtin_bit_cast(f16x8, (i32x4_)__builtin_shufflevector(a, a, 4, 5, 6, 7));
        const f16x8 bh = __builtin_bit_cast(f16x8, (i32x4_)__builtin_shufflevector(b, b, 0, 1, 2, 3));
        const f16x8 bl = __builtin_bit_cast(f16x8, (i32x4_)__builtin_shufflevector(b, b, 4, 5, 6, 7));
        acc = __builtin_amdgcn_mfma_f32_16x16x32_f16(ah, bh, acc, 0, 0, 0);
        corr = __builtin_amdgcn_mfma_f32_16x16x32_f16(ah, bl, corr, 0, 0, 0);
        corr = __builtin_amdgcn_mfma_f32_16x16x32_f16(al, bh, corr, 0, 0, 0);
    }
};
static constexpr float ST_SPLIT_INV = 1.0f / 2048.0f;
template <typename T> constexpr bool is_fp8() { return std::is_same<T, f8>::value; }
template <typename T> constexpr bool is_split() { return std::is_same<T, fsp>::value; }
template <typename T> constexpr bool frag2() { return is_fp8<T>() || is_split<T>(); }
template <typename T> struct OutT { typedef T type; };
template <> struct OutT<f8> { typedef bf16 type; };
template <> struct OutT<fsp> { typedef float type; };
template <typename T> constexpr int mfma_per_frag() { return is_split<T>() ? 3 : (sizeof(T) == 4 ? 4 : 1); }

template <typename T> struct Out4;
template <> struct Out4<bf16> {
    static __device__ __forceinline__ void load(const bf16* p, float* f) {
        bf16x4 v = *reinterpret_cast<const bf16x4*>(p);
#pragma unroll
        for (int i = 0; i < 4; ++i) f[i] = (float)v[i];
    }
    static __device__ __forceinline__ void store(bf16* p, const float* f) {
        bf16x4 v;
#pragma unroll
        for (int i = 0; i < 4; ++i) v[i] = (bf16)f[i];
        *reinterpret_cast<bf16x4*>(p) = v;
    }
};
template <> struct Out4<f16> {
    static __device__ __forceinline__ void load(const f16* p, float* f) {
        f16x4 v = *reinterpret_cast<const f16x4*>(p);
#pragma unroll
        for (int i = 0; i < 4; ++i) f[i] = (float)v[i];
    }
    static __device__ __forceinline__ void store(f16* p, const float* f) {
        f16x4 v;
#pragma unroll
        for (int i = 0; i < 4; ++i) v[i] = (f16)f[i];
        *reinterpret_cast<f16x4*>(p) = v;
    }
};
template <> struct Out4<float> {
    static __device__ __forceinline__ void load(const float* p, float* f) {
        f32x4 v = *reinterpret_cast<const f32x4*>(p);
#pragma unroll
        for (int i = 0; i < 4; ++i) f[i] = v[i];
    }
    static __device__ __forceinline__ void store(float* p, const float* f) {
        f32x4 v = {f[0], f[1], f[2], f[3]};
        *reinterpret_cast<f32x4*>(p) = v;
    }
};


__device__ __forceinline__ size_t touch_line(const GemmArgs& p, size_t l) {
    if (!p.next_row_lines) return l;
    return (l >> p.next_lead_shift) * p.next_row_lines + (l & ((1u << p.next_lead_shift) - 1u));
}
__device__ __forceinline__ void touch_next_weights(const GemmArgs& p, unsigned int& sink, bool helper = false) {
    if (!p.next_w || (p.helper_blocks > 0) != helper) return;
    const size_t lines = p.next_bytes >> 7;
    const size_t nsl = helper ? p.helper_blocks : gridDim.x;
    const size_t me = helper ? blockIdx.x - (gridDim.x - p.helper_blocks) : blockIdx.x;
    const size_t per = p.next_per ? (size_t)p.next_per : (lines + nsl - 1) / nsl;
    const size_t lo = me * per, hi = lo + per < lines ? lo + per : lines;
    const size_t step = blockDim.x;
    for (size_t l = lo + threadIdx.x; l < hi; l += step) {
        const char* a_ = (const char*)p.next_w + (touch_line(p, l) << 7);
        asm volatile("global_load_dword %0, %1, off" : "+v"(sink) : "v"(a_) : "memory");
    }
}
__device__ __forceinline__ void retire_touches(unsigned int& sink) { asm volatile("s_waitcnt vmcnt(0)" : "+v"(sink)::"memory"); }

static inline unsigned magic_u32(unsigned d) { return d <= 1 ? 0u : (unsigned)((1ull << 32) / d + 1); }
__device__ __forceinline__ int mg_div(int n, unsigned mg) { return mg ? (int)__umulhi((unsigned)n, mg) : n; }

struct TileId { int tile_m, tile_n, split, tw; };
__device__ __forceinline__ TileId tile_of_block(const GemmArgs& p, int bid, int nblk) {
    const int xq = nblk >> 3, xr = nblk & 7, xcd = bid & 7;
    const int wg = (xcd < xr ? xcd * (xq + 1) : xr * (xq + 1) + (xcd - xr) * xq) + (bid >> 3);
    TileId r;
    if (p.tm_slow) {
        r.split = wg % p.splitk; r.tw = wg / p.splitk;
        const int pn = r.tw / p.tm_per_panel, rem = r.tw - pn * p.tm_per_panel;
        const int rows = min(p.panel_h, p.tm_tiles_m - pn * p.panel_h);
        r.tile_n = rem / rows;
        r.tile_m = pn * p.panel_h + (rem - r.tile_n * rows);
        return r;
    }
    r.tw = mg_div(wg, p.tm_mg_splitk);
    r.split = wg - r.tw * p.splitk;
    const int pn = mg_div(r.tw, p.tm_mg_per_panel), rem = r.tw - pn * p.tm_per_panel;
    const bool last = (pn + 1) * p.panel_h > p.tm_tiles_m;
    const int rows = last ? p.tm_last_rows : p.panel_h;
    r.tile_n = mg_div(rem, last ? p.tm_mg_last : p.tm_mg_rows);
    r.tile_m = pn * p.panel_h + (rem - r.tile_n * rows);
    return r;
}
static inline void fill_tile_map(GemmArgs& b, int tiles_m, int tiles_n, int nk_stages) {
    const int sk = b.splitk > 1 ? b.splitk : 1;
    b.splitk = sk;
    b.tm_tiles_m = tiles_m;
    b.tm_per_panel = b.panel_h * tiles_n;
    b.tm_last_rows = tiles_m % b.panel_h ? tiles_m % b.panel_h : b.panel_h;
    b.tm_mg_splitk = magic_u32((unsigned)sk);
    b.tm_mg_per_panel = magic_u32((unsigned)b.tm_per_panel);
    b.tm_mg_rows = magic_u32((unsigned)b.panel_h);
    b.tm_mg_last = magic_u32((unsigned)b.tm_last_rows);
    const unsigned long long blocks = (unsigned long long)tiles_m * tiles_n * sk;
    b.tm_slow = (blocks * (unsigned long long)(b.tm_per_panel > sk ? b.tm_per_panel : sk) >= (1ull << 32)) ? 1 : 0;
    b.nk_base = nk_stages / sk;
    b.nk_rem = nk_stages % sk;
}
static inline void fill_next_per(GemmArgs& b, unsigned grid) {
    const size_t lines = b.next_bytes >> 7;
    const size_t nsl = b.helper_blocks > 0 ? (size_t)b.helper_blocks : (size_t)grid;
    b.next_per = (b.next_w && nsl) ? (unsigned)((lines + nsl - 1) / nsl) : 0u;
}

template <typename T> struct Raw4;
template <> struct Raw4<bf16> { typedef bf16x4 type; };
template <> struct Raw4<f16> { typedef f16x4 type; };
template <> struct Raw4<float> { typedef f32x4 type; };
template <typename T> __device__ __forceinline__ typename Raw4<T>::type ld_raw4(const T* p) {
    return *reinterpret_cast<const typename Raw4<T>::type*>(p);
}

__device__ __forceinline__ float row16_sum(float v) {
    v += __builtin_bit_cast(float, __builtin_amdgcn_update_dpp(0, __builtin_bit_cast(int, v), 0xB1, 0xF, 0xF, false));
    v += __builtin_bit_cast(float, __builtin_amdgcn_update_dpp(0, __builtin_bit_cast(int, v), 0x4E, 0xF, 0xF, false));
    v += __builtin_bit_cast(float, __builtin_amdgcn_update_dpp(0, __builtin_bit_cast(int, v), 0x124, 0xF, 0xF, false));
    v += __builtin_bit_cast(float, __builtin_amdgcn_update_dpp(0, __builtin_bit_cast(int, v), 0x128, 0xF, 0xF, false));
    return v;
}

__device__ __forceinline__ float ln_fold(float acc, float mean, float rstd, float c, float d) {
    return __builtin_fmaf(rstd, __builtin_fmaf(-mean, c, acc), d);
}

int gemm_dense_bf16(const GemmArgs& a, hipStream_t st);
int gemm_dense_f16(const GemmArgs& a, hipStream_t st);
int gemm_dense_f32(const GemmArgs& a, hipStream_t st);
int gemm_dense_f32s(const GemmArgs& a, hipStream_t st);
int gemm_dense_fp8(const GemmArgs& a, hipStream_t st);
int gemm_xattn_bf16(const GemmArgs& a, hipStream_t st);
int gemm_xattn_f16(const GemmArgs& a, hipStream_t st);
int gemm_conv_bf16(const GemmArgs& a, int R, int ups, hipStream_t st);
int gemm_conv_f16(const GemmArgs& a, int R, int ups, hipStream_t st);
int gemm_conv_f32(const GemmArgs& a, hipStream_t st);
int gemm_conv_f32s(const GemmArgs& a, int R, int ups, hipStream_t st);
int conv_thin_run(const GemmArgs& a, int R, int dtype, hipStream_t st);
```

### stabletriton_amd/csrc/gemm_dma.h

```cpp
#pragma once
#include "epilogue.h"

static __device__ __attribute__((aligned(16))) unsigned int g_zero16[4] = {0u, 0u, 0u, 0u};

typedef __attribute__((address_space(3))) void lds_void_t;
typedef __attribute__((address_space(1))) const void gbl_cvoid_t;

template <int AUX = 0>
__device__ __forceinline__ void dma16(const void* src, char* lds_wave_base) {
    __builtin_amdgcn_global_load_lds((gbl_cvoid_t*)src, (lds_void_t*)lds_wave_base, 16, 0, AUX);
}

constexpr int dma_before_last_group(int G, int NG) {
    int n = 0;
    for (int e = 0; e < G; ++e) n += (e * NG / G < NG - 1) ? 1 : 0;
    return n;
}

constexpr int dma_in_group(int G, int NG, int g) {
    int n = 0;
    for (int e = 0; e < G; ++e) n += (e * NG / G == g) ? 1 : 0;
    return n;
}

template <int AUX = 0>
__device__ __forceinline__ void dma16_at(const void* src, unsigned lds_addr) {
    __builtin_amdgcn_global_load_lds((gbl_cvoid_t*)src, (lds_void_t*)(uintptr_t)lds_addr, 16, 0, AUX);
}
__device__ __forceinline__ unsigned lds_addr_of(const char* p) { return (unsigned)(uintptr_t)(lds_void_t*)p; }

template <int N> __device__ __forceinline__ void wait_vmcnt() {
    asm volatile("s_waitcnt vmcnt(%0)" ::"n"(N) : "memory");
}


template <int TPR>
struct LnRowSum {
    static_assert(TPR == 1 || TPR == 2 || TPR == 4 || TPR == 8, "threads per row");
    static constexpr int RES = 8 / TPR;
    static constexpr int PRE = 8 / RES;
    float2 pre[RES][PRE];
    __device__ __forceinline__ void load(const float2* row, int chunks, int part) {
#pragma unroll
        for (int j = 0; j < RES; ++j)
#pragma unroll
            for (int i = 0; i < PRE; ++i) {
                const int c = part + TPR * j + 8 * i;
                pre[j][i] = row[c < chunks ? c : 0];
            }
    }
    __device__ __forceinline__ void finish(const float2* row, int chunks, int part, float& s1, float& s2) {
        float a1[RES], a2[RES];
#pragma unroll
        for (int j = 0; j < RES; ++j) {
            a1[j] = 0.f; a2[j] = 0.f;
#pragma unroll
            for (int i = 0; i < PRE; ++i) {
                const bool ok = part + TPR * j + 8 * i < chunks;
                a1[j] += ok ? pre[j][i].x : 0.f; a2[j] += ok ? pre[j][i].y : 0.f;
            }
            for (int c = part + TPR * j + 8 * PRE; c < chunks; c += 8) { const float2 v = row[c]; a1[j] += v.x; a2[j] += v.y; }
#pragma unroll
            for (int o = 1; o < TPR; o <<= 1) { a1[j] += __shfl_xor(a1[j], o, 64); a2[j] += __shfl_xor(a2[j], o, 64); }
        }
#pragma unroll
        for (int w = 1; w < RES; w <<= 1)
#pragma unroll
            for (int j = 0; j + w < RES; j += 2 * w) { a1[j] += a1[j + w]; a2[j] += a2[j + w]; }
        s1 = a1[0]; s2 = a2[0];
    }
};

template <int TM, int TN, int TILE_ELEMS>
__device__ __forceinline__ bool splitk_combine(const GemmArgs& p, f32x4 (&acc)[TM][TN], int tw, int split, char* lds, int t, int wave, int lane) {
    float* slab0 = p.partial + (size_t)tw * p.splitk * TILE_ELEMS;
    {
        asm volatile("s_nop 7\n\ts_nop 7\n\ts_nop 2" ::: "memory");
        float* mine = slab0 + (size_t)split * TILE_ELEMS + (size_t)wave * (TM * TN * 256) + lane * 4;
#pragma unroll
        for (int i = 0; i < TM; ++i)
#pragma unroll
            for (int j = 0; j < TN; ++j) {
                const float* dst = mine + (i * TN + j) * 256;
                asm volatile("global_store_dwordx4 %0, %1, off sc1\n\ts_nop 1" ::"v"(dst), "v"(acc[i][j]) : "memory");
            }
    }
    asm volatile("s_waitcnt vmcnt(0)" ::: "memory");
    __syncthreads();
    int* flag = reinterpret_cast<int*>(lds);
    if (t == 0) *flag = __hip_atomic_fetch_add(p.tile_counters + tw, 1, __ATOMIC_RELAXED, __HIP_MEMORY_SCOPE_AGENT);
    __syncthreads();
    if (*flag != p.splitk - 1) return false;
    if (t == 0) __hip_atomic_store(p.tile_counters + tw, 0, __ATOMIC_RELAXED, __HIP_MEMORY_SCOPE_AGENT);
    f32x4 own[TM][TN];
#pragma unroll
    for (int i = 0; i < TM; ++i)
#pragma unroll
        for (int j = 0; j < TN; ++j) { own[i][j] = acc[i][j]; acc[i][j] = (f32x4){0.f, 0.f, 0.f, 0.f}; }
    typedef unsigned int u32x4_ __attribute__((ext_vector_type(4)));
    const __amdgpu_buffer_rsrc_t slabs = __builtin_amdgcn_make_buffer_rsrc((void*)slab0, 0, (int)((size_t)p.splitk * TILE_ELEMS * 4), 0x00020000);
    for (int sl = 0; sl < p.splitk; ++sl) {
        if (sl == split) {
#pragma unroll
            for (int i = 0; i < TM; ++i)
#pragma unroll
                for (int j = 0; j < TN; ++j) acc[i][j] += own[i][j];
            continue;
        }
        const int off = (sl * TILE_ELEMS + wave * (TM * TN * 256) + lane * 4) * 4;
#pragma unroll
        for (int i = 0; i < TM; ++i)
#pragma unroll
            for (int j = 0; j < TN; ++j)
                acc[i][j] += __builtin_bit_cast(f32x4, (u32x4_)__builtin_amdgcn_raw_buffer_load_b128(slabs, off + (i * TN + j) * 1024, 0, 16));
    }
    return true;
}

template <typename T, int BM, int BN, int WGM, int WGN, int STAGES, int U, bool CONV, bool GEGLU, bool LNF = false, bool XA = false>
__global__ __launch_bounds__(WGM* WGN * 64) void gemm_dma_kernel(const GemmArgs p) {
    constexpr int NW = WGM * WGN;
    constexpr int VEC = 16 / (int)sizeof(T);
    constexpr int KB = 8 * VEC;
    constexpr int WTM = BM / WGM, WTN = BN / WGN;
    constexpr int TM = WTM / 16, TN = WTN / 16;
    constexpr int A_PIECES = BM / 8, B_PIECES = BN / 8;
    constexpr int A_IT = (A_PIECES + NW - 1) / NW, B_IT = (B_PIECES + NW - 1) / NW;
    constexpr bool UNEVEN = (A_PIECES % NW != 0) || (B_PIECES % NW != 0);
    constexpr int G = (A_IT + B_IT) * U;
    constexpr int A_BYTES = BM * 128, TILE = (BM + BN) * 128, STAGE = TILE * U;
    static_assert(!GEGLU || (BN % 32 == 0), "GEGLU: value and gate halves of the tile are whole 16-column accumulator tiles");
    static_assert((STAGES - 2) * G <= 63, "vmcnt immediate");
    typedef typename Mma<T>::Frag Frag;
    typedef typename OutT<T>::type TO;

    extern __shared__ __attribute__((aligned(16))) char lds[];
    char* const dump = lds + STAGES * STAGE + BM * 8;

    const int t = threadIdx.x, lane = t & 63;
    const int wave = __builtin_amdgcn_readfirstlane(t >> 6);
    const int wm = wave / WGN, wn = wave - wm * WGN;
    const int tiles_m = (p.M + BM - 1) / BM;
    const int nblk = gridDim.x - p.helper_blocks, bid = blockIdx.x;
    if (bid >= nblk) {
        unsigned int sink = 0;
        touch_next_weights(p, sink, true);
        retire_touches(sink);
        return;
    }
    constexpr int BNO = GEGLU ? BN / 2 : BN;
    const TileId tid = tile_of_block(p, bid, nblk);
    const int split = tid.split, tw = tid.tw, tile_m = tid.tile_m, tile_n = tid.tile_n;
    const int m0 = tile_m * BM;
    const int n0 = tile_n * BNO;

    const T* __restrict__ Ap = (const T*)p.A;
    const T* __restrict__ Wp = (const T*)p.W;
    const T* zeros = reinterpret_cast<const T*>(g_zero16);

    const int lr = lane >> 3;
    const int lc = (lane & 7) ^ lr;
    const T* a_ptr[A_IT];
    const T* a2_ptr[CONV ? A_IT : 1];
    int a_adv[A_IT], a_iy[A_IT], a_ix[A_IT];
#pragma unroll
    for (int i = 0; i < A_IT; ++i) {
        const int row = (wave + i * NW) * 8 + lr;
        const int m = m0 + row;
        const bool ok = m < p.M && (!UNEVEN || wave + i * NW < A_PIECES);
        if (CONV && p.A2) {
            a_ptr[i] = Ap + (size_t)(ok ? m : 0) * p.Csplit + lc * VEC;
            a2_ptr[i] = (const T*)p.A2 + (size_t)(ok ? m : 0) * (p.Cin - p.Csplit) + lc * VEC;
            a_iy[i] = ok ? 0 : -(1 << 28); a_ix[i] = 0; a_adv[i] = 0;
        } else if (CONV) {
            const int hw = p.Hout * p.Wout;
            const int mm = ok ? m : 0;
            const int img = mm / hw, rem = mm - img * hw;
            const int oy = rem / p.Wout, ox = rem - oy * p.Wout;
            a_iy[i] = ok ? oy * p.stride - p.pad : -(1 << 28);
            a_ix[i] = ox * p.stride - p.pad;
            a_ptr[i] = Ap + (size_t)img * p.Hin * p.Win * p.Cin + lc * VEC;
            a_adv[i] = 0;
        } else {
            a_ptr[i] = ok ? Ap + (size_t)m * p.lda + lc * VEC : zeros;
            a_adv[i] = ok ? KB : 0;
            a_iy[i] = a_ix[i] = 0;
        }
    }
    const T* b_ptr[B_IT];
    int b_adv[B_IT];
#pragma unroll
    for (int i = 0; i < B_IT; ++i) {
        const int row = (wave + i * NW) * 8 + lr;
        int wrow;
        bool ok;
        if (GEGLU) {
            const int half = row >= BN / 2 ? 1 : 0;
            const int ncol = n0 + row - half * (BN / 2);
            ok = ncol < p.N && (!UNEVEN || wave + i * NW < B_PIECES);
            wrow = ncol + half * p.Ng;
        } else {
            wrow = n0 + row;
            ok = wrow < p.N && (!UNEVEN || wave + i * NW < B_PIECES);
        }
        b_ptr[i] = ok ? Wp + (size_t)wrow * p.K + lc * VEC : zeros;
        b_adv[i] = ok ? KB : 0;
    }

    unsigned int touch_sink = 0;
    {
        constexpr int NT_ = NW * 64;
        const int ncols_out = min(BNO, p.N - n0);
        auto touch_at = [&](const char* a) {
            a = (const char*)((uintptr_t)a & ~(uintptr_t)3);
            asm volatile("global_load_dword %0, %1, off" : "+v"(touch_sink) : "v"(a) : "memory");
        };
        auto touch = [&](const void* base, long byte_off, int nbytes) {
            for (int o = t * 128; o < nbytes; o += NT_ * 128) touch_at((const char*)base + byte_off + o);
        };
        if (p.epi & ST_EPI_BIAS) {
            touch(p.bias, (long)n0 * sizeof(TO), ncols_out * (int)sizeof(TO));
            if (GEGLU) touch(p.bias, ((long)p.Ng + n0) * sizeof(TO), ncols_out * (int)sizeof(TO));
        }
        if (LNF) {
            touch(p.ln_c, (long)n0 * 4, ncols_out * 4); touch(p.ln_d, (long)n0 * 4, ncols_out * 4);
            if (GEGLU) { touch(p.ln_c, ((long)p.Ng + n0) * 4, ncols_out * 4); touch(p.ln_d, ((long)p.Ng + n0) * 4, ncols_out * 4); }
        }
        if (p.epi & ST_EPI_RESIDUAL) {
            const int lines = (ncols_out * (int)sizeof(TO) + 127) / 128;
            const int rows = min(BM, p.M - m0);
            for (int o = t; o < rows * lines; o += NT_) {
                const int r = o / lines, l = o - r * lines;
                touch_at((const char*)p.residual + ((size_t)(m0 + r) * p.ldr + n0) * sizeof(TO) + l * 128);
            }
        }
    }

    const int nk_lo = split * p.nk_base + min(split, p.nk_rem), nk_hi = nk_lo + p.nk_base + (split < p.nk_rem ? 1 : 0);
    const int kbase = nk_lo * U;
    constexpr int PER_TILE = A_IT + B_IT;
    int cs_r = 0, cs_s = 0, cs_c0 = 0;
    if (CONV) {
        if (p.korder) {
            const int taps = p.R_ * p.S;
            const int cs = kbase / taps, tap = kbase - cs * taps;
            cs_c0 = cs * KB; cs_r = tap / p.S; cs_s = tap - cs_r * p.S;
        } else {
            const int k0 = kbase * KB;
            const int tap = k0 / p.Cin;
            cs_c0 = k0 - tap * p.Cin; cs_r = tap / p.S; cs_s = tap - cs_r * p.S;
        }
    }
    auto conv_advance = [&](bool go) {
        if (p.korder) {
            cs_s += go ? 1 : 0;
            const bool w1 = cs_s == p.S;
            cs_s = w1 ? 0 : cs_s;
            cs_r += w1 ? 1 : 0;
            const bool w2 = cs_r == p.R_;
            cs_r = w2 ? 0 : cs_r;
            cs_c0 += w2 ? KB : 0;
        } else {
            cs_c0 += go ? KB * U : 0;
            const bool w1 = cs_c0 >= p.Cin;
            cs_c0 -= w1 ? p.Cin : 0;
            cs_s += w1 ? 1 : 0;
            const bool w2 = cs_s == p.S;
            cs_s = w2 ? 0 : cs_s;
            cs_r += w2 ? 1 : 0;
        }
    };
    const unsigned lds_base = lds_addr_of(lds), dump_addr = lds_base + STAGES * STAGE + BM * 8;
    auto issue_one = [&](int st, int buf, int e) {
        const int u = e / PER_TILE, i = e - u * PER_TILE;
        const int kt = kbase + st * U + u;
        const unsigned base = lds_base + buf * STAGE + u * TILE;
        if (i < A_IT) {
            const T* src;
            if (CONV) {
                int r, s_, c0;
                if constexpr (U == 1) {
                    r = cs_r; s_ = cs_s; c0 = cs_c0;
                } else {
                    const int k0 = kt * KB;
                    const int tap = k0 / p.Cin;
                    c0 = k0 - tap * p.Cin; r = tap / p.S; s_ = tap - r * p.S;
                }
                int iy = a_iy[i] + r, ix = a_ix[i] + s_;
                bool ok;
                if (p.ups) {
                    ok = iy >= 0 && ix >= 0 && iy < 2 * p.Hin && ix < 2 * p.Win;
                    iy >>= 1; ix >>= 1;
                } else {
                    ok = iy >= 0 && ix >= 0 && iy < p.Hin && ix < p.Win;
                }
                src = ok ? a_ptr[i] + ((size_t)iy * p.Win + ix) * p.Cin + c0 : zeros;
                if (p.A2) src = a_iy[i] < 0 ? zeros : (c0 < p.Csplit ? a_ptr[i] + c0 : a2_ptr[CONV ? i : 0] + (c0 - p.Csplit));
            } else {
                src = a_ptr[i] + (size_t)kt * a_adv[i];
            }
            const int pa = wave + i * NW;
            dma16_at<0>(src, (!UNEVEN || pa < A_PIECES) ? base + pa * 1024 : dump_addr);
        } else {
            const int j = i - A_IT;
            const int pb = wave + j * NW;
            const T* bsrc;
            if (CONV && U == 1) bsrc = b_ptr[j] + (b_adv[j] ? (size_t)((cs_r * p.S + cs_s) * p.Cin + cs_c0) : 0);
            else bsrc = b_ptr[j] + (size_t)kt * b_adv[j];
            dma16_at<0>(bsrc, (!UNEVEN || pb < B_PIECES) ? base + A_BYTES + pb * 1024 : dump_addr);
        }
    };
    auto issue = [&](int st, int buf) {
#pragma unroll
        for (int e = 0; e < G; ++e) issue_one(st, buf, e);
    };

    f32x4 acc[TM][TN];
#pragma unroll
    for (int i = 0; i < TM; ++i)
#pragma unroll
        for (int j = 0; j < TN; ++j) acc[i][j] = (f32x4){0.f, 0.f, 0.f, 0.f};

    f32x4 corr[is_split<T>() ? TM : 1][is_split<T>() ? TN : 1];
    if constexpr (is_split<T>()) {
#pragma unroll
        for (int i = 0; i < TM; ++i)
#pragma unroll
            for (int j = 0; j < TN; ++j) corr[i][j] = (f32x4){0.f, 0.f, 0.f, 0.f};
    }
    const int r16 = lane & 15, q = lane >> 4;
    const int nk = nk_hi - nk_lo;

    constexpr int TPR = (NW * 64 / BM) >= 8 ? 8 : (NW * 64 / BM >= 1 ? NW * 64 / BM : 1);
    constexpr int TPR_SPAN = NW * 64 / BM >= 1 ? NW * 64 / BM : 1;
    LnRowSum<TPR> ln_sum;
    if constexpr (LNF) {
        static_assert(NW * 64 % BM == 0 && (TPR_SPAN & (TPR_SPAN - 1)) == 0, "threads per row must be a power of two");
        const float2* st2 = reinterpret_cast<const float2*>(p.ln_stats);
        const int row = t / TPR_SPAN, part = (t - row * TPR_SPAN) & (TPR - 1);
        const int m = min(m0 + row, p.M - 1);
        ln_sum.load(st2 + (size_t)m * p.ln_chunks, p.ln_chunks, part);
    }
#pragma unroll
    for (int s_ = 0; s_ < STAGES - 1; ++s_)
        if (s_ < nk) { issue(s_, s_); if (CONV) conv_advance(s_ < nk - 1); }
    if constexpr (LNF) {
        const float2* st2 = reinterpret_cast<const float2*>(p.ln_stats);
        const int row = t / TPR_SPAN, sub = t - row * TPR_SPAN, part = sub & (TPR - 1);
        const int m = min(m0 + row, p.M - 1);
        float a1, a2;
        ln_sum.finish(st2 + (size_t)m * p.ln_chunks, p.ln_chunks, part, a1, a2);
        const float mean = a1 / (float)p.K;
        const float rstd = rsqrtf(fmaxf(a2 / (float)p.K - mean * mean, 0.f) + p.ln_eps);
        if (sub == 0) reinterpret_cast<float2*>(lds + STAGES * STAGE)[row] = make_float2(mean, rstd);
        asm volatile("s_waitcnt lgkmcnt(0)" ::: "memory");
    }
    if (nk >= STAGES - 1) wait_vmcnt<(STAGES - 2) * G>(); else wait_vmcnt<0>();
    __builtin_amdgcn_s_barrier();
    asm volatile("" ::"v"(touch_sink));

    constexpr int GPT = frag2<T>() ? 1 : 2;
    constexpr int NG = GPT * U;
    constexpr int RPF = frag2<T>() ? 2 : 1;
    constexpr bool EARLY = (STAGES == 2);
    Frag fa[2][TM], fb[2][TN];
    auto read_frag = [&](const char* base, int row, int g) -> Frag {
        if constexpr (frag2<T>()) {
            const u32x4 lo = *reinterpret_cast<const u32x4*>(base + row * 128 + ((q ^ (row & 7)) << 4));
            const u32x4 hi = *reinterpret_cast<const u32x4*>(base + row * 128 + (((q + 4) ^ (row & 7)) << 4));
            return Frag{(int)lo[0], (int)lo[1], (int)lo[2], (int)lo[3], (int)hi[0], (int)hi[1], (int)hi[2], (int)hi[3]};
        } else {
            const int c = 4 * (g & 1) + q;
            return *reinterpret_cast<const Frag*>(base + row * 128 + ((c ^ (row & 7)) << 4));
        }
    };
    auto read_group = [&](int buf, int g, int set) {
        const char* sa = lds + buf * STAGE + (g / GPT) * TILE;
        const char* sb = sa + A_BYTES;
#pragma unroll
        for (int i = 0; i < TM; ++i) fa[set][i] = read_frag(sa, wm * WTM + i * 16 + r16, g);
#pragma unroll
        for (int j = 0; j < TN; ++j) fb[set][j] = read_frag(sb, wn * WTN + j * 16 + r16, g);
    };
    auto mma_group = [&](int set) {
#pragma unroll
        for (int i = 0; i < TM; ++i)
#pragma unroll
            for (int j = 0; j < TN; ++j) {
                if constexpr (is_split<T>()) Mma<T>::run2(acc[i][j], corr[i][j], fb[set][j], fa[set][i]);
                else Mma<T>::run(acc[i][j], fb[set][j], fa[set][i]);
            }
    };

    int cur = 0, nxt = STAGES - 1;
    read_group(0, 0, 0);
    auto trip = [&](int kt, auto par_) {
        constexpr int PAR = decltype(par_)::value;
        const int pf = min(kt + STAGES - 1, nk - 1);
        auto group = [&](auto gc) {
            constexpr int g = decltype(gc)::value;
            if constexpr (g + 1 < NG) {
                read_group(cur, g + 1, (g + 1 + PAR) & 1);
            } else {
                wait_vmcnt<EARLY ? 0 : (STAGES - 3) * G + dma_before_last_group(G, NG)>();
                __builtin_amdgcn_s_barrier();
                __builtin_amdgcn_sched_barrier(0);
                read_group(cur + 1 == STAGES ? 0 : cur + 1, 0, (g + 1 + PAR) & 1);
            }
            constexpr int n_dma = EARLY ? (g == 0 ? G : 0) : dma_in_group(G, NG, g);
#pragma unroll
            for (int e = 0; e < G; ++e)
                if ((EARLY ? 0 : e * NG / G) == g) issue_one(pf, nxt, e);
            mma_group((g + PAR) & 1);
            __builtin_amdgcn_sched_group_barrier(0x100, (TM + TN) * RPF, 0);
            if constexpr (n_dma > 0) __builtin_amdgcn_sched_group_barrier(0x020, n_dma, 0);
            __builtin_amdgcn_sched_group_barrier(0x008, TM * TN * mfma_per_frag<T>(), 0);
            __builtin_amdgcn_sched_barrier(0);
        };
        group(std::integral_constant<int, 0>{});
        if constexpr (NG > 1) group(std::integral_constant<int, 1>{});
        if constexpr (NG > 2) {
            group(std::integral_constant<int, 2>{});
            group(std::integral_constant<int, 3>{});
        }
        __builtin_amdgcn_s_waitcnt(0xc07f);
        cur = cur + 1 == STAGES ? 0 : cur + 1;
        nxt = nxt + 1 == STAGES ? 0 : nxt + 1;
        if (CONV) conv_advance(kt + STAGES - 1 < nk - 1);
    };
    if constexpr (NG % 2 == 0) {
        for (int kt = 0; kt < nk; ++kt) trip(kt, std::integral_constant<int, 0>{});
    } else {
        for (int kt = 0; kt < nk; kt += 2) {
            trip(kt, std::integral_constant<int, 0>{});
            if (kt + 1 < nk) trip(kt + 1, std::integral_constant<int, 1>{});
        }
    }
    wait_vmcnt<0>();
    if constexpr (is_split<T>()) {
#pragma unroll
        for (int i = 0; i < TM; ++i)
#pragma unroll
            for (int j = 0; j < TN; ++j)
#pragma unroll
                for (int e = 0; e < 4; ++e) acc[i][j][e] = __builtin_fmaf(corr[i][j][e], ST_SPLIT_INV, acc[i][j][e]);
    }
    if (p.splitk > 1) {
        if (!splitk_combine<TM, TN, BM * BN>(p, acc, tw, split, lds, t, wave, lane)) {
            unsigned int sink = 0;
            touch_next_weights(p, sink);
            retire_touches(sink);
            return;
        }
    }
    if constexpr (XA) {
        static_assert(LNF && !GEGLU && !CONV && BM == 128 && BN == 64 && NW == 8 && sizeof(T) == 2, "xattn epilogue: 128 x 64 tile, 8 waves, 16-bit elements");
        static_assert(STAGES * STAGE >= 16384 + 3 * 16384, "xattn epilogue: Q tile + K/V ring fit the GEMM's ring");
        const float2* lnst = reinterpret_cast<const float2*>(lds + STAGES * STAGE);
        float mean[TM], rstd[TM];
#pragma unroll
        for (int i = 0; i < TM; ++i) {
            const float2 v = lnst[wm * WTM + i * 16 + r16];
            mean[i] = v.x; rstd[i] = v.y;
        }
        __syncthreads();
        T* qt = reinterpret_cast<T*>(lds);
#pragma unroll
        for (int j = 0; j < TN; ++j) {
            const int col = wn * WTN + j * 16 + 4 * q;
            const f32x4 cv = *reinterpret_cast<const f32x4*>(p.ln_c + n0 + col), dv = *reinterpret_cast<const f32x4*>(p.ln_d + n0 + col);
#pragma unroll
            for (int i = 0; i < TM; ++i) {
                const int row = wm * WTM + i * 16 + r16;
                typename V16<T>::x4 o4;
#pragma unroll
                for (int e = 0; e < 4; ++e) o4[e] = (T)ln_fold(acc[i][j][e], mean[i], rstd[i], cv[e], dv[e]);
                *reinterpret_cast<typename V16<T>::x4*>(qt + row * 64 + col) = o4;
            }
        }
        __syncthreads();
        const int bimg = m0 / p.xa_T, head = tile_n;
        const T* Kb = (const T*)p.xa_k + (size_t)bimg * p.xa_S * p.xa_ldk + (size_t)head * 64;
        const T* Vb = (const T*)p.xa_v + (size_t)bimg * p.xa_S * p.xa_ldv + (size_t)head * 64;
        attn16_core<T, 8>(qt, 64, 128, Kb, Vb, p.xa_ldk, p.xa_ldv, p.xa_S, (T*)p.C + (size_t)m0 * p.ldc + (size_t)head * 64, p.ldc,
                       min(BM, p.M - m0), p.xa_scale_log2e, lds + 16384, wave, lane);
        unsigned int sink = 0;
        touch_next_weights(p, sink);
        retire_touches(sink);
    } else if constexpr (BM * BN >= 128 * 128 || GEGLU || CONV) {
        staged_epilogue<TO, BM, BN, WGM, WGN, TM, TN, GEGLU, STAGES * STAGE, !LNF, is_fp8<T>()>(
            p, acc, m0, n0, tile_n, wm, r16, q, ColsPlain{wn, WTN}, lds, reinterpret_cast<const float2*>(lds + STAGES * STAGE));
    } else if constexpr (LNF) {
        float mean[TM], rstd[TM];
        const float2* lnst = reinterpret_cast<const float2*>(lds + STAGES * STAGE);
#pragma unroll
        for (int i = 0; i < TM; ++i) {
            const float2 v = lnst[wm * WTM + i * 16 + r16];
            mean[i] = v.x; rstd[i] = v.y;
        }
        const bool inside = (m0 + BM <= p.M) && (n0 + BNO <= p.N) && (p.N & 3) == 0 && p.C != nullptr && !p.q8_out && !p.sp_out;
        const int flags = inside ? (((p.epi & ST_EPI_BIAS) ? EPI_F_BIAS : 0) | (p.epi & (ST_EPI_RESIDUAL | ST_EPI_ROWBIAS | ST_EPI_SILU) ? 1024 : 0) |
                                    (p.col_scale ? EPI_F_SCALE : 0) | EPI_F_LN) : -1;
        if (!is_fp8<T>() && flags == EPI_F_LN) gemm_epilogue<TO, TM, TN, WTM, WTN, GEGLU, 0, 0, false, EPI_F_LN>(p, acc, m0, n0, wm, wn, r16, q, split, mean, rstd);
        else if (!is_fp8<T>() && flags == (EPI_F_LN | EPI_F_BIAS))
            gemm_epilogue<TO, TM, TN, WTM, WTN, GEGLU, 0, 0, false, EPI_F_LN | EPI_F_BIAS>(p, acc, m0, n0, wm, wn, r16, q, split, mean, rstd);
        else if (is_fp8<T>() && flags == (EPI_F_LN | EPI_F_SCALE))
            gemm_epilogue<TO, TM, TN, WTM, WTN, GEGLU, 0, 0, false, EPI_F_LN | EPI_F_SCALE>(p, acc, m0, n0, wm, wn, r16, q, split, mean, rstd);
        else gemm_epilogue<TO, TM, TN, WTM, WTN, GEGLU>(p, acc, m0, n0, wm, wn, r16, q, split, mean, rstd);
    } else {
        const bool inside = (m0 + BM <= p.M) && (n0 + BNO <= p.N) && (p.N & 3) == 0 && p.C != nullptr;
        const int flags = inside ? (((p.epi & ST_EPI_BIAS) ? EPI_F_BIAS : 0) | ((p.epi & ST_EPI_RESIDUAL) ? EPI_F_RES : 0) | ((p.epi & ST_EPI_ROWBIAS) ? EPI_F_RB : 0) |
                                    ((p.epi & ST_EPI_SILU) ? EPI_F_SILU : 0) | (p.col_scale ? EPI_F_SCALE : 0) | (p.ln_c ? EPI_F_LN : 0) | (p.row_stats ? EPI_F_ROWS : 0) |
                                    ((p.col_stats && (p.N & 3) == 0) ? EPI_F_COLS : 0) | (p.q8_out ? EPI_F_Q8 : 0) | (p.sp_out ? EPI_F_SP : 0)) : -1;
#define ST_FRAG_CASE(M)                                                                                                                        \
    case (M):                                                                                                                                  \
        gemm_epilogue<TO, TM, TN, WTM, WTN, GEGLU, WGM, WGN, false, (M)>(p, acc, m0, n0, wm, wn, r16, q, split, nullptr, nullptr, lds, tile_n); \
        break;
        bool done = false;
        if constexpr (std::is_same<TO, float>::value) {
            done = true;
            switch (flags) {
                ST_FRAG_CASE(EPI_F_BIAS | EPI_F_ROWS | EPI_F_SP)
                ST_FRAG_CASE(EPI_F_BIAS | EPI_F_RES | EPI_F_ROWS | EPI_F_SP)
                default: done = false;
            }
        }
        if (done) {
        } else if constexpr (!is_fp8<T>()) {
            switch (flags) {
                ST_FRAG_CASE(EPI_F_BIAS)
                ST_FRAG_CASE(EPI_F_BIAS | EPI_F_RES)
                ST_FRAG_CASE(EPI_F_BIAS | EPI_F_ROWS)
                ST_FRAG_CASE(EPI_F_BIAS | EPI_F_RES | EPI_F_ROWS)
                ST_FRAG_CASE(EPI_F_BIAS | EPI_F_RES | EPI_F_ROWS | EPI_F_Q8)
                ST_FRAG_CASE(EPI_F_BIAS | EPI_F_RES | EPI_F_COLS)
                default: gemm_epilogue<TO, TM, TN, WTM, WTN, GEGLU, WGM, WGN>(p, acc, m0, n0, wm, wn, r16, q, split, nullptr, nullptr, lds, tile_n);
            }
        } else {
            switch (flags) {
                ST_FRAG_CASE(EPI_F_BIAS | EPI_F_SCALE | EPI_F_RES | EPI_F_ROWS)
                ST_FRAG_CASE(EPI_F_BIAS | EPI_F_SCALE | EPI_F_RES | EPI_F_ROWS | EPI_F_Q8)
                default: gemm_epilogue<TO, TM, TN, WTM, WTN, GEGLU, WGM, WGN>(p, acc, m0, n0, wm, wn, r16, q, split, nullptr, nullptr, lds, tile_n);
            }
        }
#undef ST_FRAG_CASE
    }
}
```

### stabletriton_amd/csrc/gemm_f32.hip

```cpp
#include "gemm_core.h"

int gemm_dense_f32(const GemmArgs& a, hipStream_t st) { return gemm_dispatch<float, false>(a, st); }
int gemm_conv_f32(const GemmArgs& a, hipStream_t st) { return gemm_dispatch<float, true>(a, st); }

int conv_thin_run(const GemmArgs& a, int R, int dtype, hipStream_t st) {
    switch (dtype) {
        case ST_BF16: return conv_thin_launch<bf16>(a, R, st);
        case ST_F16: return conv_thin_launch<f16>(a, R, st);
        default: return conv_thin_launch<float>(a, R, st);
    }
}
```

### stabletriton_amd/csrc/norms.hip

```cpp
#include "common.h"
#include "split.h"
#include <type_traits>


static constexpr int GN_THREADS = 1024;
static constexpr int GN_MAX_BLOCKS = 256;

struct GnGeom {
    int VC;
    int RP;
    int NB;
    int P;
};

template <typename T>
static GnGeom gn_geom(int C, int HW) {
    GnGeom g;
    g.VC = C / Elem<T>::VEC;
    g.RP = GN_THREADS / g.VC;
    if (g.RP < 1) g.RP = 1;
    int nb = (HW + g.RP - 1) / g.RP;
    g.NB = nb < GN_MAX_BLOCKS ? nb : GN_MAX_BLOCKS;
    g.P = (HW + g.NB - 1) / g.NB;
    g.NB = (HW + g.P - 1) / g.P;
    return g;
}

template <typename T>
__global__ __launch_bounds__(GN_THREADS) void gn_stats_nhwc(const T* __restrict__ x, float4* __restrict__ part,
                                                            int C, int HW, int G, int VC, int RP, int P) {
    constexpr int VEC = Elem<T>::VEC;
    extern __shared__ __attribute__((aligned(16))) float smem[];
    const int n = blockIdx.y, b = blockIdx.x, NB = gridDim.x;
    const int t = threadIdx.x;
    const int rp = t / VC, col = t - rp * VC;
    const int p0 = b * P, p1 = min(p0 + P, HW);
    float s[VEC], ss[VEC];
#pragma unroll
    for (int i = 0; i < VEC; ++i) { s[i] = 0.f; ss[i] = 0.f; }
    if (rp < RP) {
        const T* base = x + ((size_t)n * HW) * C + (size_t)col * VEC;
        for (int p = p0 + rp; p < p1; p += RP) {
            Vec16<T> v = load16(base + (size_t)p * C);
#pragma unroll
            for (int i = 0; i < VEC; ++i) { float f = v.get(i); s[i] += f; ss[i] += f * f; }
        }
        float* row = smem + (size_t)rp * 2 * C;
#pragma unroll
        for (int i = 0; i < VEC; ++i) { row[col * VEC + i] = s[i]; row[C + col * VEC + i] = ss[i]; }
    }
    __syncthreads();
    for (int c = t; c < 2 * C; c += GN_THREADS) {
        float a = 0.f;
        for (int r = 0; r < RP; ++r) a += smem[(size_t)r * 2 * C + c];
        smem[c] = a;
    }
    __syncthreads();
    if (t < G) {
        const int cpg = C / G;
        float S = 0.f, SS = 0.f;
        for (int i = 0; i < cpg; ++i) { S += smem[t * cpg + i]; SS += smem[C + t * cpg + i]; }
        const float cnt = (float)(max(p1 - p0, 0)) * (float)cpg;
        float mean = cnt > 0.f ? S / cnt : 0.f;
        float m2 = cnt > 0.f ? fmaxf(SS - S * mean, 0.f) : 0.f;
        part[((size_t)n * NB + b) * G + t] = make_float4(mean, m2, cnt, 0.f);
    }
}

template <typename T>
__global__ __launch_bounds__(256) void gn_stats_nchw(const T* __restrict__ x, float4* __restrict__ part,
                                                     int C, int HW, int G, long chunk) {
    const int ng = blockIdx.y, b = blockIdx.x, NB = gridDim.x;
    const int n = ng / G, g = ng - n * G;
    const int cpg = C / G;
    const long total = (long)cpg * HW;
    const T* base = x + ((size_t)n * C + (size_t)g * cpg) * HW;
    const long i0 = (long)b * chunk, i1 = min(i0 + chunk, total);
    float s = 0.f, ss = 0.f;
    for (long i = i0 + threadIdx.x; i < i1; i += 256) { float f = Elem<T>::to_f(base[i]); s += f; ss += f * f; }
    __shared__ float red[2][4];
    s = wave_sum(s); ss = wave_sum(ss);
    if ((threadIdx.x & 63) == 0) { red[0][threadIdx.x >> 6] = s; red[1][threadIdx.x >> 6] = ss; }
    __syncthreads();
    if (threadIdx.x == 0) {
        float S = red[0][0] + red[0][1] + red[0][2] + red[0][3];
        float SS = red[1][0] + red[1][1] + red[1][2] + red[1][3];
        float cnt = (float)max(i1 - i0, 0L);
        float mean = cnt > 0.f ? S / cnt : 0.f;
        float m2 = cnt > 0.f ? fmaxf(SS - S * mean, 0.f) : 0.f;
        part[((size_t)n * NB + b) * G + g] = make_float4(mean, m2, cnt, 0.f);
    }
}

__device__ __forceinline__ void chan_merge(float& mean, float& m2, float& cnt, float pm, float p2, float pc) {
    const float tot = cnt + pc;
    if (pc > 0.f) {
        const float d = pm - mean;
        const float w = pc / tot;
        mean += d * w;
        m2 += p2 + d * d * (cnt * w);
        cnt = tot;
    }
}

__global__ __launch_bounds__(256) void gn_finalize(const float4* __restrict__ part, float2* __restrict__ stats, int NB, int G, int NG, float eps) {
    const int i = blockIdx.x * 4 + (threadIdx.x >> 6);
    const int lane = threadIdx.x & 63;
    if (i >= NG) return;
    const int n = i / G, g = i - n * G;
    float mean = 0.f, m2 = 0.f, cnt = 0.f;
    for (int b = lane; b < NB; b += 64) {
        const float4 p = part[((size_t)n * NB + b) * G + g];
        chan_merge(mean, m2, cnt, p.x, p.y, p.z);
    }
#pragma unroll
    for (int o = 1; o < 64; o <<= 1) {
        const float pm = __shfl_xor(mean, o, 64), p2 = __shfl_xor(m2, o, 64), pc = __shfl_xor(cnt, o, 64);
        const bool low = (lane & o) == 0;
        float am = low ? mean : pm, a2 = low ? m2 : p2, ac = low ? cnt : pc;
        const float bm = low ? pm : mean, b2 = low ? p2 : m2, bc = low ? pc : cnt;
        chan_merge(am, a2, ac, bm, b2, bc);
        mean = am; m2 = a2; cnt = ac;
    }
    if (lane == 0) stats[i] = make_float2(mean, rsqrtf(m2 / cnt + eps));
}

template <typename T, bool SILU>
__global__ __launch_bounds__(GN_THREADS) void gn_apply_nhwc(const T* __restrict__ x, const T* __restrict__ gamma,
                                                            const T* __restrict__ beta, const float2* __restrict__ stats,
                                                            T* __restrict__ y, int C, int HW, int G, int VC, int RP, int P,
                                                            const T* __restrict__ x1 = nullptr, int C0 = 0, char* __restrict__ ys = nullptr) {
    constexpr int VEC = Elem<T>::VEC;
    const int n = blockIdx.y, b = blockIdx.x;
    const int t = threadIdx.x;
    const int rp = t / VC, col = t - rp * VC;
    if (rp >= RP) return;
    const int p0 = b * P, p1 = min(p0 + P, HW);
    const int cpg = C / G;
    float mu[VEC], a[VEC], bt[VEC];
    Vec16<T> gv = load16(gamma + col * VEC), bv = load16(beta + col * VEC);
#pragma unroll
    for (int i = 0; i < VEC; ++i) {
        float2 st = stats[n * G + (col * VEC + i) / cpg];
        mu[i] = st.x; a[i] = st.y * gv.get(i); bt[i] = bv.get(i);
    }
    const size_t base = ((size_t)n * HW) * C + (size_t)col * VEC;
    const bool second = x1 != nullptr && col * VEC >= C0;
    const int Cs = x1 == nullptr ? C : (second ? C - C0 : C0);
    const T* __restrict__ xs = (second ? x1 + ((size_t)n * HW) * Cs + (size_t)(col * VEC - C0) : x + ((size_t)n * HW) * Cs + (size_t)col * VEC);
    for (int p = p0 + rp; p < p1; p += RP) {
        Vec16<T> v = load16(xs + (size_t)p * Cs), o;
#pragma unroll
        for (int i = 0; i < VEC; ++i) {
            float f = (v.get(i) - mu[i]) * a[i] + bt[i];
            if (SILU) f = silu_f(f);
            o.set(i, f);
        }
        store16(y + base + (size_t)p * C, o);
        if constexpr (std::is_same<T, float>::value) {
            if (ys) {
                const float v4[4] = {o.get(0), o.get(1), o.get(2), o.get(3)};
                split_store4(ys + ((size_t)n * HW + p) * C * 4, col * VEC, v4);
            }
        }
    }
}

template <typename T, bool SILU>
__global__ __launch_bounds__(256) void gn_apply_nchw(const T* __restrict__ x, const T* __restrict__ gamma,
                                                     const T* __restrict__ beta, const float2* __restrict__ stats,
                                                     T* __restrict__ y, int C, int HW, int G) {
    const int nc = blockIdx.y;
    const int n = nc / C, c = nc - n * C;
    const float2 st = stats[n * G + c / (C / G)];
    const float a = st.y * Elem<T>::to_f(gamma[c]), bt = Elem<T>::to_f(beta[c]);
    const size_t base = (size_t)nc * HW;
    for (int i = blockIdx.x * 256 + threadIdx.x; i < HW; i += gridDim.x * 256) {
        float f = (Elem<T>::to_f(x[base + i]) - st.x) * a + bt;
        if (SILU) f = silu_f(f);
        y[base + i] = Elem<T>::from_f(f);
    }
}

static size_t gn_ws_bytes(int N, int G) {
    return (size_t)N * GN_MAX_BLOCKS * G * sizeof(float4) + (size_t)N * G * sizeof(float2);
}

template <typename T>
static int gn_launch(const void* x, const void* gamma, const void* beta, void* y, int N, int C, int HW, int G,
                     float eps, int silu, int layout, void* ws, hipStream_t st, char* ys = nullptr) {
    float4* part = (float4*)ws;
    float2* stats = (float2*)((char*)ws + (size_t)N * GN_MAX_BLOCKS * G * sizeof(float4));
    int NB;
    if (layout == ST_NHWC) {
        ST_REQUIRE(C % Elem<T>::VEC == 0, "group_norm NHWC: C=%d must be a multiple of %d", C, Elem<T>::VEC);
        GnGeom g = gn_geom<T>(C, HW);
        ST_REQUIRE(g.VC <= GN_THREADS, "group_norm NHWC: C=%d too wide", C);
        size_t lds = (size_t)g.RP * 2 * C * sizeof(float);
        ST_REQUIRE(lds <= 160 * 1024, "group_norm NHWC: LDS %zu too large", lds);
        NB = g.NB;
        hipLaunchKernelGGL(gn_stats_nhwc<T>, dim3(NB, N), dim3(GN_THREADS), lds, st, (const T*)x, part, C, HW, G, g.VC, g.RP, g.P);
        hipLaunchKernelGGL(gn_finalize, dim3(cdiv(N * G, 4)), dim3(256), 0, st, part, stats, NB, G, N * G, eps);
        if (silu)
            hipLaunchKernelGGL((gn_apply_nhwc<T, true>), dim3(NB, N), dim3(GN_THREADS), 0, st, (const T*)x, (const T*)gamma,
                               (const T*)beta, stats, (T*)y, C, HW, G, g.VC, g.RP, g.P, (const T*)nullptr, 0, ys);
        else
            hipLaunchKernelGGL((gn_apply_nhwc<T, false>), dim3(NB, N), dim3(GN_THREADS), 0, st, (const T*)x, (const T*)gamma,
                               (const T*)beta, stats, (T*)y, C, HW, G, g.VC, g.RP, g.P, (const T*)nullptr, 0, ys);
    } else {
        const long total = (long)(C / G) * HW;
        NB = (int)((total + 8191) / 8192);
        if (NB > GN_MAX_BLOCKS) NB = GN_MAX_BLOCKS;
        int want = cdiv(1024, N * G);
        if (NB > want && want >= 1) NB = want > 1 ? want : 1;
        long chunk = (total + NB - 1) / NB;
        NB = (int)((total + chunk - 1) / chunk);
        hipLaunchKernelGGL(gn_stats_nchw<T>, dim3(NB, N * G), dim3(256), 0, st, (const T*)x, part, C, HW, G, chunk);
        hipLaunchKernelGGL(gn_finalize, dim3(cdiv(N * G, 4)), dim3(256), 0, st, part, stats, NB, G, N * G, eps);
        int bx = cdiv(HW, 256 * 4);
        if (bx < 1) bx = 1;
        if (silu)
            hipLaunchKernelGGL((gn_apply_nchw<T, true>), dim3(bx, N * C), dim3(256), 0, st, (const T*)x, (const T*)gamma,
                               (const T*)beta, stats, (T*)y, C, HW, G);
        else
            hipLaunchKernelGGL((gn_apply_nchw<T, false>), dim3(bx, N * C), dim3(256), 0, st, (const T*)x, (const T*)gamma,
                               (const T*)beta, stats, (T*)y, C, HW, G);
    }
    return st_check_launch("group_norm");
}

extern "C" size_t st_group_norm_workspace_bytes(int N, int C, int HW, int groups) {
    (void)C; (void)HW;
    return gn_ws_bytes(N, groups);
}

extern "C" int st_group_norm(const void* x, const void* gamma, const void* beta, void* y, int N, int C, int HW,
                             int groups, float eps, int silu, int layout, int dtype, void* workspace, void* stream) {
    ST_REQUIRE(x && gamma && beta && y && workspace, "group_norm: null pointer");
    ST_REQUIRE(N > 0 && C > 0 && HW > 0 && groups > 0 && C % groups == 0, "group_norm: bad shape N=%d C=%d HW=%d G=%d", N, C, HW, groups);
    ST_REQUIRE(groups <= 1024 && N * C <= 65535 && N <= 65535, "group_norm: shape exceeds launch limits");
    ST_REQUIRE(layout == ST_NCHW || layout == ST_NHWC, "group_norm: bad layout %d", layout);
    hipStream_t st = (hipStream_t)stream;
    void* ys = nullptr;
    if (int e = st_take_split_arm("group_norm", (long)N * HW, C, dtype == ST_F32 && layout == ST_NHWC && C % 32 == 0, &ys)) return e;
    if (dtype == ST_BF16) return gn_launch<bf16>(x, gamma, beta, y, N, C, HW, groups, eps, silu, layout, workspace, st);
    if (dtype == ST_F16) return gn_launch<f16>(x, gamma, beta, y, N, C, HW, groups, eps, silu, layout, workspace, st);
    if (dtype == ST_F32) return gn_launch<float>(x, gamma, beta, y, N, C, HW, groups, eps, silu, layout, workspace, st, (char*)ys);
    return st_fail("group_norm: unsupported dtype %d", dtype);
}

struct GnSource { const float2* part; int C; int tiles_per_image; };

__global__ __launch_bounds__(256) void gn_cols_finalize(GnSource s0, GnSource s1, float2* __restrict__ stats, int G, int NG,
                                                        int cpg, double count, float eps) {
    const int i = blockIdx.x, t_ = threadIdx.x;
    const int n = i / G, g = i - n * G;
    const int c_lo = g * cpg;
    double S = 0.0, Q = 0.0;
    auto sweep = [&](const GnSource& src, int lo, int hi) {
        const int w = hi - lo;
        if (w <= 0) return;
        const float2* base = src.part + (size_t)n * src.tiles_per_image * src.C + lo;
        const int total = w * src.tiles_per_image;
        for (int k = t_; k < total; k += 256) {
            const int t = k / w, c = k - t * w;
            const float2 v = base[(size_t)t * src.C + c];
            S += (double)v.x; Q += (double)v.y;
        }
    };
    const int c_hi = c_lo + cpg;
    sweep(s0, min(c_lo, s0.C), min(c_hi, s0.C));
    sweep(s1, max(c_lo, s0.C) - s0.C, max(c_hi, s0.C) - s0.C);
    __shared__ double red[2][4];
#pragma unroll
    for (int o = 32; o > 0; o >>= 1) { S += __shfl_xor(S, o, 64); Q += __shfl_xor(Q, o, 64); }
    if ((t_ & 63) == 0) { red[0][t_ >> 6] = S; red[1][t_ >> 6] = Q; }
    __syncthreads();
    if (t_ == 0) {
        S = (red[0][0] + red[0][1]) + (red[0][2] + red[0][3]);
        Q = (red[1][0] + red[1][1]) + (red[1][2] + red[1][3]);
        const double mean = S / count;
        const double var = fmax(Q / count - mean * mean, 0.0);
        stats[i] = make_float2((float)mean, (float)(1.0 / sqrt(var + (double)eps)));
    }
    (void)NG;
}

template <typename T>
static int gn_from_stats_launch(const void* x, const void* gamma, const void* beta, void* y, int N, int C, int HW, int G, float eps,
                                int silu, GnSource s0, GnSource s1, void* ws, hipStream_t st, const void* x1 = nullptr, int C0 = 0,
                                char* ys = nullptr) {
    ST_REQUIRE(C % Elem<T>::VEC == 0, "group_norm_from_stats: C=%d must be a multiple of %d", C, Elem<T>::VEC);
    GnGeom g = gn_geom<T>(C, HW);
    ST_REQUIRE(g.VC <= GN_THREADS, "group_norm_from_stats: C=%d too wide", C);
    float2* stats = (float2*)ws;
    hipLaunchKernelGGL(gn_cols_finalize, dim3(N * G), dim3(256), 0, st, s0, s1, stats, G, N * G, C / G,
                       (double)(C / G) * (double)HW, eps);
    if (silu)
        hipLaunchKernelGGL((gn_apply_nhwc<T, true>), dim3(g.NB, N), dim3(GN_THREADS), 0, st, (const T*)x, (const T*)gamma,
                           (const T*)beta, stats, (T*)y, C, HW, G, g.VC, g.RP, g.P, (const T*)x1, C0, ys);
    else
        hipLaunchKernelGGL((gn_apply_nhwc<T, false>), dim3(g.NB, N), dim3(GN_THREADS), 0, st, (const T*)x, (const T*)gamma,
                           (const T*)beta, stats, (T*)y, C, HW, G, g.VC, g.RP, g.P, (const T*)x1, C0, ys);
    return st_check_launch("group_norm_from_stats");
}

extern "C" int st_group_norm_from_stats(const void* x, const void* gamma, const void* beta, void* y, int N, int C, int HW,
                                        int groups, float eps, int silu, int dtype, const float* stats0, int C0, int rows0,
                                        const float* stats1, int C1, int rows1, void* workspace, void* stream) {
    ST_REQUIRE(x && gamma && beta && y && workspace && stats0, "group_norm_from_stats: null pointer");
    ST_REQUIRE(N > 0 && C > 0 && HW > 0 && groups > 0 && C % groups == 0, "group_norm_from_stats: bad shape N=%d C=%d HW=%d G=%d", N, C, HW, groups);
    ST_REQUIRE(groups <= 1024 && N <= 65535, "group_norm_from_stats: shape exceeds launch limits");
    ST_REQUIRE(C0 > 0 && rows0 > 0 && HW % rows0 == 0, "group_norm_from_stats: source 0 has %d rows per partial for HW=%d", rows0, HW);
    ST_REQUIRE((stats1 == nullptr && C1 == 0 && C0 == C) || (stats1 && C1 > 0 && rows1 > 0 && HW % rows1 == 0 && C0 + C1 == C),
               "group_norm_from_stats: sources cover %d + %d channels, input has %d", C0, C1, C);
    GnSource s0 = {(const float2*)stats0, C0, HW / rows0};
    GnSource s1 = {(const float2*)stats1, C1, stats1 ? HW / rows1 : 0};
    hipStream_t st = (hipStream_t)stream;
    void* ys = nullptr;
    if (int e = st_take_split_arm("group_norm_from_stats", (long)N * HW, C, dtype == ST_F32 && C % 32 == 0, &ys)) return e;
    if (dtype == ST_BF16) return gn_from_stats_launch<bf16>(x, gamma, beta, y, N, C, HW, groups, eps, silu, s0, s1, workspace, st);
    if (dtype == ST_F16) return gn_from_stats_launch<f16>(x, gamma, beta, y, N, C, HW, groups, eps, silu, s0, s1, workspace, st);
    if (dtype == ST_F32) return gn_from_stats_launch<float>(x, gamma, beta, y, N, C, HW, groups, eps, silu, s0, s1, workspace, st, nullptr, 0, (char*)ys);
    return st_fail("group_norm_from_stats: unsupported dtype %d", dtype);
}

extern "C" int st_group_norm_from_stats_cat(const void* x0, const void* x1, const void* gamma, const void* beta, void* y, int N, int C, int HW,
                                            int groups, float eps, int silu, int dtype, const float* stats0, int C0, int rows0,
                                            const float* stats1, int C1, int rows1, void* workspace, void* stream) {
    ST_REQUIRE(x0 && x1 && gamma && beta && y && workspace && stats0 && stats1, "group_norm_from_stats_cat: null pointer");
    ST_REQUIRE(N > 0 && C > 0 && HW > 0 && groups > 0 && C % groups == 0, "group_norm_from_stats_cat: bad shape N=%d C=%d HW=%d G=%d", N, C, HW, groups);
    ST_REQUIRE(groups <= 1024 && N <= 65535, "group_norm_from_stats_cat: shape exceeds launch limits");
    ST_REQUIRE(C0 > 0 && C1 > 0 && C0 + C1 == C && rows0 > 0 && rows1 > 0 && HW % rows0 == 0 && HW % rows1 == 0,
               "group_norm_from_stats_cat: sources cover %d + %d channels, input has %d", C0, C1, C);
    const int vec = dtype == ST_F32 ? 4 : 8;
    ST_REQUIRE(C0 % vec == 0 && C1 % vec == 0, "group_norm_from_stats_cat: channel counts (%d, %d) must be multiples of %d", C0, C1, vec);
    GnSource s0 = {(const float2*)stats0, C0, HW / rows0};
    GnSource s1 = {(const float2*)stats1, C1, HW / rows1};
    hipStream_t st = (hipStream_t)stream;
    void* ys = nullptr;
    if (int e = st_take_split_arm("group_norm_from_stats_cat", (long)N * HW, C, dtype == ST_F32 && C % 32 == 0, &ys)) return e;
    if (dtype == ST_BF16) return gn_from_stats_launch<bf16>(x0, gamma, beta, y, N, C, HW, groups, eps, silu, s0, s1, workspace, st, x1, C0);
    if (dtype == ST_F16) return gn_from_stats_launch<f16>(x0, gamma, beta, y, N, C, HW, groups, eps, silu, s0, s1, workspace, st, x1, C0);
    if (dtype == ST_F32) return gn_from_stats_launch<float>(x0, gamma, beta, y, N, C, HW, groups, eps, silu, s0, s1, workspace, st, x1, C0, (char*)ys);
    return st_fail("group_norm_from_stats_cat: unsupported dtype %d", dtype);
}

template <typename T, int NV>
__global__ __launch_bounds__(256) void ln_kernel(const T* __restrict__ x, const T* __restrict__ gamma,
                                                 const T* __restrict__ beta, T* __restrict__ y, int rows, int C, float eps) {
    constexpr int VEC = Elem<T>::VEC;
    const int lane = threadIdx.x & 63;
    const int row = blockIdx.x * 4 + (threadIdx.x >> 6);
    if (row >= rows) return;
    const int VC = C / VEC;
    const T* xr = x + (size_t)row * C;
    Vec16<T> v[NV];
    float s = 0.f;
#pragma unroll
    for (int j = 0; j < NV; ++j) {
        const int vc = lane + 64 * j;
        if (vc < VC) {
            v[j] = load16(xr + vc * VEC);
#pragma unroll
            for (int i = 0; i < VEC; ++i) s += v[j].get(i);
        }
    }
    const float mean = wave_sum(s) / (float)C;
    float q = 0.f;
#pragma unroll
    for (int j = 0; j < NV; ++j) {
        if (lane + 64 * j < VC) {
#pragma unroll
            for (int i = 0; i < VEC; ++i) { float d = v[j].get(i) - mean; q += d * d; }
        }
    }
    const float rstd = rsqrtf(wave_sum(q) / (float)C + eps);
    T* yr = y + (size_t)row * C;
#pragma unroll
    for (int j = 0; j < NV; ++j) {
        const int vc = lane + 64 * j;
        if (vc < VC) {
            Vec16<T> g = load16(gamma + vc * VEC), b = load16(beta + vc * VEC), o;
#pragma unroll
            for (int i = 0; i < VEC; ++i) o.set(i, (v[j].get(i) - mean) * rstd * g.get(i) + b.get(i));
            store16(yr + vc * VEC, o);
        }
    }
}

template <typename T>
static int ln_launch(const void* x, const void* g, const void* b, void* y, int rows, int C, float eps, hipStream_t st) {
    constexpr int VEC = Elem<T>::VEC;
    ST_REQUIRE(C % VEC == 0, "layer_norm: C=%d must be a multiple of %d", C, VEC);
    const int nv = cdiv(C / VEC, 64);
    ST_REQUIRE(nv <= 8, "layer_norm: C=%d too wide", C);
    dim3 grid(cdiv(rows, 4)), block(256);
#define LN_CASE(NV) case NV: hipLaunchKernelGGL((ln_kernel<T, NV>), grid, block, 0, st, (const T*)x, (const T*)g, (const T*)b, (T*)y, rows, C, eps); break;
    switch (nv) { LN_CASE(1) LN_CASE(2) LN_CASE(3) LN_CASE(4) LN_CASE(5) LN_CASE(6) LN_CASE(7) LN_CASE(8) }
#undef LN_CASE
    return st_check_launch("layer_norm");
}

extern "C" int st_layer_norm(const void* x, const void* gamma, const void* beta, void* y, int rows, int C, float eps,
                             int dtype, void* stream) {
    ST_REQUIRE(x && gamma && beta && y, "layer_norm: null pointer");
    ST_REQUIRE(rows > 0 && C > 0, "layer_norm: bad shape rows=%d C=%d", rows, C);
    hipStream_t st = (hipStream_t)stream;
    if (dtype == ST_BF16) return ln_launch<bf16>(x, gamma, beta, y, rows, C, eps, st);
    if (dtype == ST_F16) return ln_launch<f16>(x, gamma, beta, y, rows, C, eps, st);
    if (dtype == ST_F32) return ln_launch<float>(x, gamma, beta, y, rows, C, eps, st);
    return st_fail("layer_norm: unsupported dtype %d", dtype);
}

template <typename T>
__global__ __launch_bounds__(256) void geglu_kernel(const T* __restrict__ state, const T* __restrict__ gate, T* __restrict__ out,
                                                    long nvec, int FV, long lds_, long ldg, long ldo) {
    constexpr int VEC = Elem<T>::VEC;
    for (long i = (long)blockIdx.x * 256 + threadIdx.x; i < nvec; i += (long)gridDim.x * 256) {
        const long r = i / FV;
        const int c = (int)(i - r * FV) * VEC;
        Vec16<T> a = load16(state + r * lds_ + c), g = load16(gate + r * ldg + c), o;
#pragma unroll
        for (int k = 0; k < VEC; ++k) o.set(k, a.get(k) * gelu_for<T>(g.get(k)));
        store16(out + r * ldo + c, o);
    }
}

template <typename T>
static int geglu_launch(const void* s, const void* g, void* o, int rows, int F, long lds_, long ldg, long ldo, hipStream_t st) {
    constexpr int VEC = Elem<T>::VEC;
    ST_REQUIRE(F % VEC == 0 && lds_ % VEC == 0 && ldg % VEC == 0 && ldo % VEC == 0,
               "geglu: F and row strides must be multiples of %d", VEC);
    ST_REQUIRE(((uintptr_t)s | (uintptr_t)g | (uintptr_t)o) % 16 == 0, "geglu: pointers must be 16-byte aligned");
    const long nvec = (long)rows * (F / VEC);
    int grid = (int)((nvec + 255) / 256);
    if (grid > 4096) grid = 4096;
    hipLaunchKernelGGL(geglu_kernel<T>, dim3(grid), dim3(256), 0, st, (const T*)s, (const T*)g, (T*)o, nvec, F / VEC, lds_, ldg, ldo);
    return st_check_launch("geglu");
}

extern "C" int st_geglu(const void* state, const void* gate, void* out, int rows, int F, long ld_state, long ld_gate,
                        long ld_out, int dtype, void* stream) {
    ST_REQUIRE(state && gate && out, "geglu: null pointer");
    ST_REQUIRE(rows > 0 && F > 0, "geglu: bad shape rows=%d F=%d", rows, F);
    hipStream_t st = (hipStream_t)stream;
    if (dtype == ST_BF16) return geglu_launch<bf16>(state, gate, out, rows, F, ld_state, ld_gate, ld_out, st);
    if (dtype == ST_F16) return geglu_launch<f16>(state, gate, out, rows, F, ld_state, ld_gate, ld_out, st);
    if (dtype == ST_F32) return geglu_launch<float>(state, gate, out, rows, F, ld_state, ld_gate, ld_out, st);
    return st_fail("geglu: unsupported dtype %d", dtype);
}
```

Measured before the change: 76.37 it/s.

## Add stem/thin-out conv kernels, dense 1x1 conv path, fused GN stats-apply

Adds a specialised stem conv kernel for Cin=4 3x3, a thin-output conv kernel for Cout of 4 or 8 that reduces across lanes, and routes 1x1 convs and concat 1x1 convs through the dense GEMM path with a concat-A variant. It also folds the group-norm stats finalize into the apply kernel so that launch is dropped, and unrolls the apply loop by four. These target several small, poorly utilised kernels and extra launches, at the cost of more template variants and new dispatch conditions.

```diff
diff --git a/stabletriton_amd/csrc/conv_thin.h b/stabletriton_amd/csrc/conv_thin.h
--- a/stabletriton_amd/csrc/conv_thin.h
+++ b/stabletriton_amd/csrc/conv_thin.h
@@ -89,7 +89,94 @@
 }
 
 template <typename T>
+__global__ __launch_bounds__(256) void conv_stem_kernel(const GemmArgs p) {
+    extern __shared__ __attribute__((aligned(16))) float wsm[];
+    const T* x = (const T*)p.A;
+    const T* w = (const T*)p.W;
+    constexpr int K = 36;
+    const int N = p.N;
+    for (int i = threadIdx.x; i < K * N; i += 256) {
+        const int nl = i / K, k = i - nl * K;
+        wsm[k * N + nl] = Elem<T>::to_f(w[i]);
+    }
+    __syncthreads();
+    const int lane = threadIdx.x & 63, wave = threadIdx.x >> 6;
+    const int oct = lane & 7;
+    const int He = p.ups ? 2 * p.Hin : p.Hin, We = p.ups ? 2 * p.Win : p.Win;
+    const int hw = p.Hout * p.Wout;
+#pragma unroll 1
+    for (int h = 0; h < 2; ++h) {
+        const int m = (blockIdx.x * 4 + wave) * 16 + h * 8 + (lane >> 3);
+        if (m >= p.M) continue;
+        const int img = m / hw, rem = m - img * hw;
+        const int oy = rem / p.Wout, ox = rem - oy * p.Wout;
+        float xin[K];
+#pragma unroll
+        for (int r = 0; r < 3; ++r)
+#pragma unroll
+            for (int s_ = 0; s_ < 3; ++s_) {
+                int iy = oy * p.stride - p.pad + r, ix = ox * p.stride - p.pad + s_;
+                const bool ok = iy >= 0 && ix >= 0 && iy < He && ix < We;
+                if (p.ups) { iy >>= 1; ix >>= 1; }
+                const T* xp = x + (((size_t)img * p.Hin + (ok ? iy : 0)) * p.Win + (ok ? ix : 0)) * 4;
+                float f[4];
+                Out4<T>::load(xp, f);
+#pragma unroll
+                for (int c = 0; c < 4; ++c) xin[(r * 3 + s_) * 4 + c] = ok ? f[c] : 0.f;
+            }
+#pragma unroll 1
+        for (int n0 = oct * 8; n0 < N; n0 += 64) {
+            float v[8];
+#pragma unroll
+            for (int e = 0; e < 8; ++e) v[e] = 0.f;
+#pragma unroll
+            for (int k = 0; k < K; ++k) {
+                const f32x4 wa = *reinterpret_cast<const f32x4*>(wsm + k * N + n0), wb = *reinterpret_cast<const f32x4*>(wsm + k * N + n0 + 4);
+#pragma unroll
+                for (int e = 0; e < 4; ++e) { v[e] += xin[k] * wa[e]; v[4 + e] += xin[k] * wb[e]; }
+            }
+            if (p.epi & ST_EPI_BIAS) {
+#pragma unroll
+                for (int e = 0; e < 8; ++e) v[e] += Elem<T>::to_f(((const T*)p.bias)[n0 + e]);
+            }
+            if (p.epi & ST_EPI_SILU) {
+#pragma unroll
+                for (int e = 0; e < 8; ++e) v[e] = silu_f(v[e]);
+            }
+            if (p.epi & ST_EPI_ROWBIAS) {
+#pragma unroll
+                for (int e = 0; e < 8; ++e) v[e] += Elem<T>::to_f(((const T*)p.rowbias)[(size_t)(m / p.rows_per_batch) * N + n0 + e]);
+            }
+            if (p.epi & ST_EPI_RESIDUAL) {
+#pragma unroll
+                for (int e = 0; e < 8; ++e) v[e] += Elem<T>::to_f(((const T*)p.residual)[(size_t)m * p.ldr + n0 + e]);
+            }
+            T* out = (T*)p.C + (size_t)m * p.ldc + n0;
+            if constexpr (Elem<T>::VEC == 8) {
+                Vec16<T> o;
+#pragma unroll
+                for (int e = 0; e < 8; ++e) o.set(e, v[e]);
+                store16(out, o);
+            } else {
+                Out4<T>::store(out, v);
+                Out4<T>::store(out + 4, v + 4);
+            }
+        }
+    }
+}
+
+template <typename T>
+static bool conv_stem_applies(const GemmArgs& a, int R) {
+    return R == 3 && a.S == 3 && a.Cin == 4 && a.N % 64 == 0 && (size_t)36 * a.N * sizeof(float) <= 64 * 1024 &&
+           a.ldc % 8 == 0 && ((uintptr_t)a.C & 15) == 0 && ((uintptr_t)a.A & 7) == 0;
+}
+
+template <typename T>
 static int conv_thin_launch(const GemmArgs& a, int R, hipStream_t st) {
+    if (conv_stem_applies<T>(a, R)) {
+        hipLaunchKernelGGL((conv_stem_kernel<T>), dim3(cdiv(a.M, 64)), dim3(256), (size_t)36 * a.N * sizeof(float), st, a);
+        return st_check_launch("conv2d(stem)");
+    }
     const int bx = cdiv(a.M, 256);
     int ny = cdiv(1024, bx);
     if (ny > a.N / 16) ny = a.N / 16;
@@ -101,3 +188,107 @@
     hipLaunchKernelGGL((conv_thin_kernel<T, 64>), dim3(bx, ny), dim3(256), lds, st, a, R, chunk);
     return st_check_launch("conv2d(thin)");
 }
+
+template <typename T, int COUT, int CH>
+__global__ __launch_bounds__(256) void conv_thin_out_kernel(const GemmArgs p, int R, int NCV) {
+    constexpr int VEC = Elem<T>::VEC;
+    constexpr int WSTR = COUT * VEC + 4;
+    extern __shared__ __attribute__((aligned(16))) float wsm[];
+    const T* __restrict__ x = (const T*)p.A;
+    const T* __restrict__ w = (const T*)p.W;
+    const int K = p.K, Cin = p.Cin, taps = R * p.S;
+    for (int i = threadIdx.x; i < K * COUT; i += 256) {
+        const int co = i / K, k = i - co * K;
+        const int tap = k / Cin, c = k - tap * Cin;
+        const int cv = c / VEC, e = c - cv * VEC;
+        wsm[(tap * NCV + cv) * WSTR + co * VEC + e] = Elem<T>::to_f(w[i]);
+    }
+    __syncthreads();
+    const int lane = threadIdx.x & 63, wave = threadIdx.x >> 6;
+    const int cvl = lane & 7;
+    const int m = (blockIdx.x * 4 + wave) * 8 + (lane >> 3);
+    const bool live = m < p.M;
+    const int mm = live ? m : 0;
+    const int hw = p.Hout * p.Wout;
+    const int img = mm / hw, rem = mm - img * hw;
+    const int oy = rem / p.Wout, ox = rem - oy * p.Wout;
+    const int He = p.ups ? 2 * p.Hin : p.Hin, We = p.ups ? 2 * p.Win : p.Win;
+    const int nit = NCV / 8;
+    float acc[COUT];
+#pragma unroll
+    for (int co = 0; co < COUT; ++co) acc[co] = 0.f;
+    int tap = 0;
+    for (int r = 0; r < R; ++r)
+        for (int s_ = 0; s_ < p.S; ++s_, ++tap) {
+            int iy = oy * p.stride - p.pad + r, ix = ox * p.stride - p.pad + s_;
+            const bool ok = live && iy >= 0 && ix >= 0 && iy < He && ix < We;
+            if (p.ups) { iy >>= 1; ix >>= 1; }
+            const T* xp = x + (((size_t)img * p.Hin + (ok ? iy : 0)) * p.Win + (ok ? ix : 0)) * Cin + cvl * VEC;
+            const float* wt = wsm + (size_t)(tap * NCV + cvl) * WSTR;
+            for (int i0 = 0; i0 < nit; i0 += CH) {
+                Vec16<T> v[CH];
+#pragma unroll
+                for (int u = 0; u < CH; ++u) {
+                    const bool in = ok && i0 + u < nit;
+                    if (in) v[u] = load16(xp + (size_t)(i0 + u) * 8 * VEC);
+                    else {
+#pragma unroll
+                        for (int e = 0; e < VEC; ++e) v[u].set(e, 0.f);
+                    }
+                }
+#pragma unroll
+                for (int u = 0; u < CH; ++u) {
+                    if (i0 + u < nit) {
+                        const float* wp = wt + (size_t)(i0 + u) * 8 * WSTR;
+#pragma unroll
+                        for (int e0 = 0; e0 < VEC; e0 += 4) {
+                            const float x0 = v[u].get(e0), x1 = v[u].get(e0 + 1), x2 = v[u].get(e0 + 2), x3 = v[u].get(e0 + 3);
+#pragma unroll
+                            for (int co = 0; co < COUT; ++co) {
+                                const f32x4 w4 = *reinterpret_cast<const f32x4*>(wp + co * VEC + e0);
+                                acc[co] += x0 * w4[0]; acc[co] += x1 * w4[1]; acc[co] += x2 * w4[2]; acc[co] += x3 * w4[3];
+                            }
+                        }
+                    }
+                }
+            }
+        }
+#pragma unroll
+    for (int co = 0; co < COUT; ++co) {
+        float a = acc[co];
+        a += __shfl_xor(a, 1, 64); a += __shfl_xor(a, 2, 64); a += __shfl_xor(a, 4, 64);
+        acc[co] = a;
+    }
+    if (!live || cvl != 0) return;
+#pragma unroll
+    for (int c0 = 0; c0 < COUT; c0 += 4) {
+        float v4[4] = {acc[c0], acc[c0 + 1], acc[c0 + 2], acc[c0 + 3]};
+        if (p.epi & ST_EPI_BIAS)
+            for (int e = 0; e < 4; ++e) v4[e] += Elem<T>::to_f(((const T*)p.bias)[c0 + e]);
+        Out4<T>::store((T*)p.C + (size_t)m * p.ldc + c0, v4);
+    }
+}
+
+template <typename T>
+static bool conv_thin_out_applies(const GemmArgs& a, int R) {
+    constexpr int VEC = Elem<T>::VEC;
+    if ((a.N != 4 && a.N != 8) || a.Cin % (8 * VEC) != 0 || (a.epi & ~ST_EPI_BIAS) || a.col_stats || a.sp_out || a.A2) return false;
+    return (size_t)R * a.S * (a.Cin / VEC) * (a.N * VEC + 4) * sizeof(float) <= 64 * 1024;
+}
+
+template <typename T>
+static int conv_thin_out_launch(const GemmArgs& a, int R, hipStream_t st) {
+    constexpr int VEC = Elem<T>::VEC;
+    const int ncv = a.Cin / VEC;
+    const size_t lds = (size_t)R * a.S * ncv * (a.N * VEC + 4) * sizeof(float);
+    const dim3 grid(cdiv(a.M, 32));
+    const bool five = (ncv / 8) % 5 == 0;
+    if (a.N == 4) {
+        if (five) hipLaunchKernelGGL((conv_thin_out_kernel<T, 4, 5>), grid, dim3(256), lds, st, a, R, ncv);
+        else hipLaunchKernelGGL((conv_thin_out_kernel<T, 4, 4>), grid, dim3(256), lds, st, a, R, ncv);
+    } else {
+        if (five) hipLaunchKernelGGL((conv_thin_out_kernel<T, 8, 5>), grid, dim3(256), lds, st, a, R, ncv);
+        else hipLaunchKernelGGL((conv_thin_out_kernel<T, 8, 4>), grid, dim3(256), lds, st, a, R, ncv);
+    }
+    return st_check_launch("conv2d(thin out)");
+}
diff --git a/stabletriton_amd/csrc/dispatch.h b/stabletriton_amd/csrc/dispatch.h
--- a/stabletriton_amd/csrc/dispatch.h
+++ b/stabletriton_amd/csrc/dispatch.h
@@ -21,11 +21,11 @@
     return ok;
 }
 
-template <typename T, int BM, int BN, int WGM, int WGN, int STAGES, int U, bool CONV, bool GEGLU, bool LNF, bool XA = false>
+template <typename T, int BM, int BN, int WGM, int WGN, int STAGES, int U, bool CONV, bool GEGLU, bool LNF, bool XA = false, bool CAT = false>
 static void launch_dma_one(const GemmArgs& a, hipStream_t st, int tiles_n) {
     const size_t lds = (size_t)STAGES * U * (BM + BN) * 128 + (size_t)BM * 8 + 1024;
     const int sk = a.splitk > 1 ? a.splitk : 1;
-    auto kfn = gemm_dma_kernel<T, BM, BN, WGM, WGN, STAGES, U, CONV, GEGLU, LNF, XA>;
+    auto kfn = gemm_dma_kernel<T, BM, BN, WGM, WGN, STAGES, U, CONV, GEGLU, LNF, XA, CAT>;
     const bool emit_cols = colstats_ok(a, BM, LNF);
     static unsigned long long lds_ok = 0;
     ensure_dynamic_lds(kfn, lds, &lds_ok);
@@ -55,9 +55,18 @@
     hipLaunchKernelGGL(kfn, dim3(main_blocks + b.helper_blocks), dim3(WGM * WGN * 64), lds, st, b);
 }
 
+template <typename T, int BM, int BN, int NW, int STAGES, int U> constexpr bool cat_tile() {
+    return !is_fp8<T>() && BN != 320 && !(is_split<T>() && BM == 256) && NW == 8 && U == 1 && STAGES >= 3;
+}
+
 template <typename T, int BM, int BN, int WGM, int WGN, int STAGES, int U, bool CONV>
 static void launch_dma(const GemmArgs& a, hipStream_t st) {
     if constexpr (!CONV) {
+        if (a.A2) {
+            if constexpr (cat_tile<T, BM, BN, WGM * WGN, STAGES, U>() || std::is_same<T, float>::value)
+                launch_dma_one<T, BM, BN, WGM, WGN, STAGES, U, false, false, false, false, true>(a, st, cdiv(a.N, BN));
+            return;
+        }
         const bool geglu = a.epi & ST_EPI_GEGLU;
         constexpr bool PAIRS = (BN % 32 == 0);
         if (a.ln_c) {
@@ -77,6 +86,8 @@
 enum { CFG_64x64_S4 = 0, CFG_64x64_S8 = 1, CFG_64x64_S4_U2 = 2, CFG_128x64_S4 = 3, CFG_128x64_S3_U2 = 4,
        CFG_128x128_S3 = 5, CFG_64x64_S3 = 6, CFG_64x64_W8 = 7, CFG_128x64_W8 = 8, CFG_128x128_W8 = 9,
        CFG_64x128_W8 = 10, CFG_64x128_W8_S6 = 11, CFG_128x64_W8_S6 = 12, CFG_128x128_W8_S4 = 13, CFG_64x64_W8_S8 = 14, CFG_64x128_W8_U2 = 15, CFG_128x64_W8_U2 = 16, CFG_64x64_W8_U2 = 17, CFG_256x256_W8 = 18, CFG_256x128_W8 = 19, CFG_128x128_W8_S2 = 20, CFG_128x64_W8_S3 = 21, CFG_64x128_W8_S3 = 22, CFG_128x320_W8 = 23, CFG_128x256_W8 = 24, CFG_64x320_W8 = 25, CFG_64x80_W4 = 26, CFG_128x80_W8 = 27, CFG_128x160_W8 = 28, CFG_128x128_N4_S2 = 29, CFG_128x64_N4_S3 = 30, CFG_64x128_N4_S3 = 31, CFG_256x160_W8_S2 = 32, CFG_COUNT, CFG_256x256_8P = 100, CFG_256x160_8P = 101, CFG_256x256_4W = 102 };
+
+static inline bool cat_cfg(int cfg) { return cfg != CFG_128x320_W8 && cfg != CFG_64x320_W8; }
 
 static inline int cfg_bn(int cfg) {
     switch (cfg) {
@@ -186,6 +197,7 @@
                 if (frag2<T>() && c.bn == 320) continue;
                 if (is_split<T>() && c.cfg == CFG_256x128_W8) continue;
                 if ((a.epi & ST_EPI_GEGLU) && c.bn % 32 != 0) continue;
+                if (a.dense_1x1 && !cat_cfg(c.cfg)) continue;
                 const long nt = tiles_(c.bm, c.bn);
                 const double trip = (is_split<T>() && c.cfg == CFG_128x160_W8 ? ST_SPLIT_160_TRIP : c.trip_us * (is_split<T>() && !CONV ? ST_SPLIT_DENSE_TRIP : 1.0)) * (CONV ? 1.6 : 1.0) * ((!CONV && sizeof(T) == 2) ? model_tweak(c.cfg) : 1.0);
                 for (int k_ : sks) {
@@ -208,7 +220,7 @@
             if (gemm8p_applies(a, 256, KB)) c256 = (double)((tiles(256, 256) + 255) / 256) * (nk * 1.65 + 4.0);
             if (gemm8p_applies(a, 160, KB)) c160 = (double)((tiles(256, 160) + 255) / 256) * (nk * 1.52 + 4.0);
 #ifdef ST_DEV_CONFIGS
-            if (f == CFG_256x256_4W && gemm4w_applies(a, KB)) { gemm4w_call<T>(a, st); return st_check_launch(who); }
+            if (f == CFG_256x256_4W && !a.dense_1x1 && gemm4w_applies(a, KB)) { gemm4w_call<T>(a, st); return st_check_launch(who); }
 #endif
             static const bool no_colsplit = dev_env_int("ST_NO_COLSPLIT", 0) != 0;
             if (f < 0 && depth == 0 && !no_colsplit && c256 < 1e29 && !a.row_stats && !a.col_stats && !a.q8_out && !a.sp_out && !a.row_scale) {
@@ -256,7 +268,7 @@
 #ifdef ST_DEV_CONFIGS
         {
             static const int small_cfg = dev_env_int("ST_GEMM_SMALL_CFG", -1);
-            if (small_cfg >= 0 && small_cfg < CFG_COUNT && tiles(128, 128) < 150 && sk == 1) cfg = small_cfg;
+            if (small_cfg >= 0 && small_cfg < CFG_COUNT && tiles(128, 128) < 150 && sk == 1 && !a.dense_1x1) cfg = small_cfg;
         }
 #endif
         {
@@ -266,7 +278,7 @@
             if (g_dbg_cfg >= 0) force_fk = g_dbg_fusek;
 #endif
             const int f = forced_cfg();
-            if (f >= 0 && f < CFG_COUNT) {
+            if (f >= 0 && f < CFG_COUNT && !a.dense_1x1) {
                 const bool u2 = (f == CFG_64x64_S4_U2 || f == CFG_128x64_S3_U2 || f == CFG_64x128_W8_U2 || f == CFG_128x64_W8_U2 ||
                                  f == CFG_64x64_W8_U2);
                 if (!u2 || even2) { cfg = f; sk = (force_fk > 1 && can_split) ? (force_fk > nk ? nk : force_fk) : 1; }
diff --git a/stabletriton_amd/csrc/gemm8p.h b/stabletriton_amd/csrc/gemm8p.h
--- a/stabletriton_amd/csrc/gemm8p.h
+++ b/stabletriton_amd/csrc/gemm8p.h
@@ -252,7 +252,7 @@
 
 static inline bool gemm8p_applies(const GemmArgs& a, int bn, int kb = 64) {
     const long n_rows = (a.epi & ST_EPI_GEGLU) ? 2L * a.N : a.N;
-    return a.M % 256 == 0 && n_rows % bn == 0 && a.K % kb == 0 && a.K >= 2 * kb && a.N % 8 == 0 &&
+    return !a.dense_1x1 && a.M % 256 == 0 && n_rows % bn == 0 && a.K % kb == 0 && a.K >= 2 * kb && a.N % 8 == 0 &&
            !(a.epi & ST_EPI_ROWBIAS) && (!a.row_stats || !(a.epi & ST_EPI_GEGLU));
 }
 
diff --git a/stabletriton_amd/csrc/gemm_api.hip b/stabletriton_amd/csrc/gemm_api.hip
--- a/stabletriton_amd/csrc/gemm_api.hip
+++ b/stabletriton_amd/csrc/gemm_api.hip
@@ -171,6 +171,8 @@
     return gemm_dense_fp8(a, (hipStream_t)stream);
 }
 
+static bool conv1x1_dense(const GemmArgs& a) { return !a.col_stats || a.rows_per_batch % 256 == 0; }
+
 extern "C" int st_conv2d(const void* x, const void* W, const void* bias, const void* residual, const void* rowbias, void* y,
                          int N, int Hin, int Win, int Cin, int Cout, int R, int S, int stride, int pad, int upsample2x,
                          int epilogue, int dtype, void* workspace, size_t workspace_bytes,
@@ -205,6 +207,11 @@
     const int kb = st_dtype_is16(dtype) ? 64 : 32;
     if (Cin % kb == 0) {
         ST_REQUIRE(((uintptr_t)x | (uintptr_t)W | (uintptr_t)y) % 16 == 0, "conv2d: pointers must be 16-byte aligned");
+        if (R == 1 && S == 1 && stride == 1 && pad == 0 && !upsample2x && conv1x1_dense(a)) {
+            a.lda = Cin; a.dense_1x1 = 1;
+            return run_dense(a, dtype, st);
+        }
+        if (conv_thin_out_takes(a, R, dtype)) return conv_thin_out_run(a, R, dtype, st);
         if (dtype == ST_BF16) return gemm_conv_bf16(a, R, upsample2x, st);
         if (dtype == ST_F16) return gemm_conv_f16(a, R, upsample2x, st);
         if (dtype == ST_F32S) return gemm_conv_f32s(a, R, upsample2x, st);
@@ -240,6 +247,10 @@
     if (int e = check_epilogue("conv1x1_cat", a)) return e;
     if (int e = st_take_split_arm("conv1x1_cat", a.M, Cout, !st_dtype_is16(dtype) && Cout % 32 == 0, &a.sp_out)) return e;
     hipStream_t st = (hipStream_t)stream;
+    if (conv1x1_dense(a)) {
+        a.lda = C0; a.dense_1x1 = 1;
+        return run_dense(a, dtype, st);
+    }
     if (dtype == ST_BF16) return gemm_conv_bf16(a, 1, 0, st);
     if (dtype == ST_F16) return gemm_conv_f16(a, 1, 0, st);
     if (dtype == ST_F32S) return gemm_conv_f32s(a, 1, 0, st);
diff --git a/stabletriton_amd/csrc/gemm_args.h b/stabletriton_amd/csrc/gemm_args.h
--- a/stabletriton_amd/csrc/gemm_args.h
+++ b/stabletriton_amd/csrc/gemm_args.h
@@ -25,6 +25,7 @@
     int* tile_counters;
     int panel_h;
     const void* A2; int Csplit;
+    int dense_1x1;
     int tm_tiles_m, tm_per_panel, tm_last_rows, tm_slow;
     unsigned tm_mg_splitk, tm_mg_per_panel, tm_mg_rows, tm_mg_last;
     int nk_base, nk_rem;
@@ -241,3 +242,5 @@
 int gemm_conv_f32(const GemmArgs& a, hipStream_t st);
 int gemm_conv_f32s(const GemmArgs& a, int R, int ups, hipStream_t st);
 int conv_thin_run(const GemmArgs& a, int R, int dtype, hipStream_t st);
+bool conv_thin_out_takes(const GemmArgs& a, int R, int dtype);
+int conv_thin_out_run(const GemmArgs& a, int R, int dtype, hipStream_t st);
diff --git a/stabletriton_amd/csrc/gemm_dma.h b/stabletriton_amd/csrc/gemm_dma.h
--- a/stabletriton_amd/csrc/gemm_dma.h
+++ b/stabletriton_amd/csrc/gemm_dma.h
@@ -117,8 +117,9 @@
     return true;
 }
 
-template <typename T, int BM, int BN, int WGM, int WGN, int STAGES, int U, bool CONV, bool GEGLU, bool LNF = false, bool XA = false>
+template <typename T, int BM, int BN, int WGM, int WGN, int STAGES, int U, bool CONV, bool GEGLU, bool LNF = false, bool XA = false, bool CAT = false>
 __global__ __launch_bounds__(WGM* WGN * 64) void gemm_dma_kernel(const GemmArgs p) {
+    static_assert(!CAT || (!CONV && !GEGLU && !LNF && !XA), "two-source A: the plain dense kernel only");
     constexpr int NW = WGM * WGN;
     constexpr int VEC = 16 / (int)sizeof(T);
     constexpr int KB = 8 * VEC;
@@ -161,7 +162,7 @@
     const int lr = lane >> 3;
     const int lc = (lane & 7) ^ lr;
     const T* a_ptr[A_IT];
-    const T* a2_ptr[CONV ? A_IT : 1];
+    const T* a2_ptr[(CONV || CAT) ? A_IT : 1];
     int a_adv[A_IT], a_iy[A_IT], a_ix[A_IT];
 #pragma unroll
     for (int i = 0; i < A_IT; ++i) {
@@ -185,6 +186,7 @@
             a_ptr[i] = ok ? Ap + (size_t)m * p.lda + lc * VEC : zeros;
             a_adv[i] = ok ? KB : 0;
             a_iy[i] = a_ix[i] = 0;
+            if constexpr (CAT) a2_ptr[i] = ok ? (const T*)p.A2 + (size_t)m * (p.K - p.Csplit) + lc * VEC : zeros;
         }
     }
     const T* b_ptr[B_IT];
@@ -296,6 +298,9 @@
                 }
                 src = ok ? a_ptr[i] + ((size_t)iy * p.Win + ix) * p.Cin + c0 : zeros;
                 if (p.A2) src = a_iy[i] < 0 ? zeros : (c0 < p.Csplit ? a_ptr[i] + c0 : a2_ptr[CONV ? i : 0] + (c0 - p.Csplit));
+            } else if constexpr (CAT) {
+                const int ks = p.Csplit / KB;
+                src = kt < ks ? a_ptr[i] + (size_t)kt * a_adv[i] : a2_ptr[i] + (size_t)(kt - ks) * a_adv[i];
             } else {
                 src = a_ptr[i] + (size_t)kt * a_adv[i];
             }
diff --git a/stabletriton_amd/csrc/gemm_f32.hip b/stabletriton_amd/csrc/gemm_f32.hip
--- a/stabletriton_amd/csrc/gemm_f32.hip
+++ b/stabletriton_amd/csrc/gemm_f32.hip
@@ -10,3 +10,20 @@
         default: return conv_thin_launch<float>(a, R, st);
     }
 }
+
+bool conv_thin_out_takes(const GemmArgs& a, int R, int dtype) {
+    switch (dtype) {
+        case ST_BF16: return conv_thin_out_applies<bf16>(a, R);
+        case ST_F16: return conv_thin_out_applies<f16>(a, R);
+        case ST_F32: return conv_thin_out_applies<float>(a, R);
+        default: return false;
+    }
+}
+
+int conv_thin_out_run(const GemmArgs& a, int R, int dtype, hipStream_t st) {
+    switch (dtype) {
+        case ST_BF16: return conv_thin_out_launch<bf16>(a, R, st);
+        case ST_F16: return conv_thin_out_launch<f16>(a, R, st);
+        default: return conv_thin_out_launch<float>(a, R, st);
+    }
+}
diff --git a/stabletriton_amd/csrc/norms.hip b/stabletriton_amd/csrc/norms.hip
--- a/stabletriton_amd/csrc/norms.hip
+++ b/stabletriton_amd/csrc/norms.hip
@@ -1,5 +1,6 @@
 #include "common.h"
 #include "split.h"
+#include <stdlib.h>
 #include <type_traits>
 
 
@@ -125,31 +126,114 @@
     if (lane == 0) stats[i] = make_float2(mean, rsqrtf(m2 / cnt + eps));
 }
 
-template <typename T, bool SILU>
+struct GnSource { const float2* part; int C; int tiles_per_image; };
+
+static inline int gn_dev_env_int(const char* name, int dflt) {
+#ifdef ST_DEV_CONFIGS
+    const char* e = getenv(name);
+    return e ? atoi(e) : dflt;
+#else
+    (void)name;
+    return dflt;
+#endif
+}
+
+static constexpr int GN_FUSE_TEAMS = GN_THREADS / 256;
+static constexpr int GN_FUSE_NJ = 4;
+static constexpr int GN_FUSE_MAXG = 256;
+
+template <int NJ, int TEAMS>
+__device__ __forceinline__ void gn_cols_stats(const GnSource& s0, const GnSource& s1, int n, int g_first, int g_stride, int G, int cpg,
+                                              double count, float eps, int tt, int team, double* __restrict__ red, float2* __restrict__ out) {
+    const float2* const img0 = s0.part + (size_t)n * s0.tiles_per_image * s0.C;
+    const float2* const img1 = s1.part + (size_t)n * s1.tiles_per_image * s1.C;
+    auto range = [&](int j, int s, int& w, int& total) -> unsigned {
+        const int g = g_first + j * g_stride;
+        const int c_lo = g * cpg, c_hi = c_lo + cpg;
+        const int lo = s ? max(c_lo, s0.C) - s0.C : min(c_lo, s0.C);
+        const int hi = s ? max(c_hi, s0.C) - s0.C : min(c_hi, s0.C);
+        w = g < G ? max(hi - lo, 0) : 0;
+        total = w * (s ? s1 : s0).tiles_per_image;
+        return (unsigned)lo;
+    };
+    float2 first[NJ][2];
+#pragma unroll
+    for (int j = 0; j < NJ; ++j)
+#pragma unroll
+        for (int s = 0; s < 2; ++s) {
+            int w, total;
+            const unsigned base = range(j, s, w, total);
+            first[j][s] = make_float2(0.f, 0.f);
+            if (tt < total) {
+                const int t = tt / w, c = tt - t * w;
+                first[j][s] = (s ? img1 : img0)[base + (unsigned)(t * (s ? s1.C : s0.C) + c)];
+            }
+        }
+#pragma unroll
+    for (int j = 0; j < NJ; ++j) {
+        double S = 0.0, Q = 0.0;
+#pragma unroll
+        for (int s = 0; s < 2; ++s) {
+            int w, total;
+            const unsigned base = range(j, s, w, total);
+            if (tt < total) { S += (double)first[j][s].x; Q += (double)first[j][s].y; }
+            for (int k = tt + 256; k < total; k += 256) {
+                const int t = k / w, c = k - t * w;
+                const float2 v = (s ? img1 : img0)[base + (unsigned)(t * (s ? s1.C : s0.C) + c)];
+                S += (double)v.x; Q += (double)v.y;
+            }
+        }
+#pragma unroll
+        for (int o = 32; o > 0; o >>= 1) { S += __shfl_xor(S, o, 64); Q += __shfl_xor(Q, o, 64); }
+        if ((tt & 63) == 0) { red[((team * NJ + j) * 2 + 0) * 4 + (tt >> 6)] = S; red[((team * NJ + j) * 2 + 1) * 4 + (tt >> 6)] = Q; }
+        __builtin_amdgcn_sched_barrier(0);
+    }
+    __syncthreads();
+    if (tt < NJ && g_first + tt * g_stride < G) {
+        const double* r = red + (team * NJ + tt) * 8;
+        const double S = (r[0] + r[1]) + (r[2] + r[3]);
+        const double Q = (r[4] + r[5]) + (r[6] + r[7]);
+        const double mean = S / count;
+        const double var = fmax(Q / count - mean * mean, 0.0);
+        out[g_first + tt * g_stride] = make_float2((float)mean, (float)(1.0 / sqrt(var + (double)eps)));
+    }
+}
+
+template <typename T, bool SILU, bool FUSED = false>
 __global__ __launch_bounds__(GN_THREADS) void gn_apply_nhwc(const T* __restrict__ x, const T* __restrict__ gamma,
                                                             const T* __restrict__ beta, const float2* __restrict__ stats,
                                                             T* __restrict__ y, int C, int HW, int G, int VC, int RP, int P,
-                                                            const T* __restrict__ x1 = nullptr, int C0 = 0, char* __restrict__ ys = nullptr) {
+                                                            const T* __restrict__ x1 = nullptr, int C0 = 0, char* __restrict__ ys = nullptr,
+                                                            GnSource s0 = {}, GnSource s1 = {}, double count = 0.0, float eps = 0.f) {
     constexpr int VEC = Elem<T>::VEC;
     const int n = blockIdx.y, b = blockIdx.x;
     const int t = threadIdx.x;
+    const int cpg = C / G;
+    __shared__ double red[FUSED ? GN_FUSE_TEAMS * GN_FUSE_NJ * 8 : 1];
+    __shared__ float2 st_lds[FUSED ? GN_FUSE_MAXG : 1];
+    if constexpr (FUSED) {
+        for (int g0 = 0; g0 < G; g0 += GN_FUSE_TEAMS * GN_FUSE_NJ) {
+            gn_cols_stats<GN_FUSE_NJ, GN_FUSE_TEAMS>(s0, s1, n, g0 + (t >> 8), GN_FUSE_TEAMS, G, cpg, count, eps, t & 255, t >> 8, red, st_lds);
+            __syncthreads();
+        }
+    }
+    const float2* const st_of = FUSED ? st_lds : stats + n * G;
     const int rp = t / VC, col = t - rp * VC;
     if (rp >= RP) return;
     const int p0 = b * P, p1 = min(p0 + P, HW);
-    const int cpg = C / G;
     float mu[VEC], a[VEC], bt[VEC];
     Vec16<T> gv = load16(gamma + col * VEC), bv = load16(beta + col * VEC);
 #pragma unroll
     for (int i = 0; i < VEC; ++i) {
-        float2 st = stats[n * G + (col * VEC + i) / cpg];
+        float2 st = st_of[(col * VEC + i) / cpg];
         mu[i] = st.x; a[i] = st.y * gv.get(i); bt[i] = bv.get(i);
     }
     const size_t base = ((size_t)n * HW) * C + (size_t)col * VEC;
     const bool second = x1 != nullptr && col * VEC >= C0;
     const int Cs = x1 == nullptr ? C : (second ? C - C0 : C0);
     const T* __restrict__ xs = (second ? x1 + ((size_t)n * HW) * Cs + (size_t)(col * VEC - C0) : x + ((size_t)n * HW) * Cs + (size_t)col * VEC);
-    for (int p = p0 + rp; p < p1; p += RP) {
-        Vec16<T> v = load16(xs + (size_t)p * Cs), o;
+    auto one = [&](int p, const Vec16<T>& v) {
+        Vec16<T> o;
 #pragma unroll
         for (int i = 0; i < VEC; ++i) {
             float f = (v.get(i) - mu[i]) * a[i] + bt[i];
@@ -163,7 +247,14 @@
                 split_store4(ys + ((size_t)n * HW + p) * C * 4, col * VEC, v4);
             }
         }
-    }
+    };
+    int p = p0 + rp;
+    for (; p + 3 * RP < p1; p += 4 * RP) {
+        const Vec16<T> v0 = load16(xs + (size_t)p * Cs), v1 = load16(xs + (size_t)(p + RP) * Cs);
+        const Vec16<T> v2 = load16(xs + (size_t)(p + 2 * RP) * Cs), v3 = load16(xs + (size_t)(p + 3 * RP) * Cs);
+        one(p, v0); one(p + RP, v1); one(p + 2 * RP, v2); one(p + 3 * RP, v3);
+    }
+    for (; p < p1; p += RP) one(p, load16(xs + (size_t)p * Cs));
 }
 
 template <typename T, bool SILU>
@@ -203,10 +294,10 @@
         hipLaunchKernelGGL(gn_finalize, dim3(cdiv(N * G, 4)), dim3(256), 0, st, part, stats, NB, G, N * G, eps);
         if (silu)
             hipLaunchKernelGGL((gn_apply_nhwc<T, true>), dim3(NB, N), dim3(GN_THREADS), 0, st, (const T*)x, (const T*)gamma,
-                               (const T*)beta, stats, (T*)y, C, HW, G, g.VC, g.RP, g.P, (const T*)nullptr, 0, ys);
+                               (const T*)beta, stats, (T*)y, C, HW, G, g.VC, g.RP, g.P, (const T*)nullptr, 0, ys, GnSource{}, GnSource{}, 0.0, 0.f);
         else
             hipLaunchKernelGGL((gn_apply_nhwc<T, false>), dim3(NB, N), dim3(GN_THREADS), 0, st, (const T*)x, (const T*)gamma,
-                               (const T*)beta, stats, (T*)y, C, HW, G, g.VC, g.RP, g.P, (const T*)nullptr, 0, ys);
+                               (const T*)beta, stats, (T*)y, C, HW, G, g.VC, g.RP, g.P, (const T*)nullptr, 0, ys, GnSource{}, GnSource{}, 0.0, 0.f);
     } else {
         const long total = (long)(C / G) * HW;
         NB = (int)((total + 8191) / 8192);
@@ -249,42 +340,16 @@
     return st_fail("group_norm: unsupported dtype %d", dtype);
 }
 
-struct GnSource { const float2* part; int C; int tiles_per_image; };
-
 __global__ __launch_bounds__(256) void gn_cols_finalize(GnSource s0, GnSource s1, float2* __restrict__ stats, int G, int NG,
                                                         int cpg, double count, float eps) {
-    const int i = blockIdx.x, t_ = threadIdx.x;
+    __shared__ double red[8];
+    const int i = blockIdx.x;
     const int n = i / G, g = i - n * G;
-    const int c_lo = g * cpg;
-    double S = 0.0, Q = 0.0;
-    auto sweep = [&](const GnSource& src, int lo, int hi) {
-        const int w = hi - lo;
-        if (w <= 0) return;
-        const float2* base = src.part + (size_t)n * src.tiles_per_image * src.C + lo;
-        const int total = w * src.tiles_per_image;
-        for (int k = t_; k < total; k += 256) {
-            const int t = k / w, c = k - t * w;
-            const float2 v = base[(size_t)t * src.C + c];
-            S += (double)v.x; Q += (double)v.y;
-        }
-    };
-    const int c_hi = c_lo + cpg;
-    sweep(s0, min(c_lo, s0.C), min(c_hi, s0.C));
-    sweep(s1, max(c_lo, s0.C) - s0.C, max(c_hi, s0.C) - s0.C);
-    __shared__ double red[2][4];
-#pragma unroll
-    for (int o = 32; o > 0; o >>= 1) { S += __shfl_xor(S, o, 64); Q += __shfl_xor(Q, o, 64); }
-    if ((t_ & 63) == 0) { red[0][t_ >> 6] = S; red[1][t_ >> 6] = Q; }
-    __syncthreads();
-    if (t_ == 0) {
-        S = (red[0][0] + red[0][1]) + (red[0][2] + red[0][3]);
-        Q = (red[1][0] + red[1][1]) + (red[1][2] + red[1][3]);
-        const double mean = S / count;
-        const double var = fmax(Q / count - mean * mean, 0.0);
-        stats[i] = make_float2((float)mean, (float)(1.0 / sqrt(var + (double)eps)));
-    }
+    gn_cols_stats<1, 1>(s0, s1, n, g, 1, G, cpg, count, eps, threadIdx.x, 0, red, stats + (size_t)n * G);
     (void)NG;
 }
+
+static constexpr size_t GN_FUSE_MAX_BYTES = 200 * 1024;
 
 template <typename T>
 static int gn_from_stats_launch(const void* x, const void* gamma, const void* beta, void* y, int N, int C, int HW, int G, float eps,
@@ -294,14 +359,26 @@
     GnGeom g = gn_geom<T>(C, HW);
     ST_REQUIRE(g.VC <= GN_THREADS, "group_norm_from_stats: C=%d too wide", C);
     float2* stats = (float2*)ws;
-    hipLaunchKernelGGL(gn_cols_finalize, dim3(N * G), dim3(256), 0, st, s0, s1, stats, G, N * G, C / G,
-                       (double)(C / G) * (double)HW, eps);
+    const double count = (double)(C / G) * (double)HW;
+    const size_t part_bytes = ((size_t)s0.tiles_per_image * s0.C + (size_t)s1.tiles_per_image * s1.C) * sizeof(float2);
+    static const int force = gn_dev_env_int("ST_GN_FUSE", -1);
+    const bool fuse = G <= GN_FUSE_MAXG && (force >= 0 ? force != 0 : part_bytes <= GN_FUSE_MAX_BYTES);
+    if (fuse) {
+        if (silu)
+            hipLaunchKernelGGL((gn_apply_nhwc<T, true, true>), dim3(g.NB, N), dim3(GN_THREADS), 0, st, (const T*)x, (const T*)gamma,
+                               (const T*)beta, (const float2*)nullptr, (T*)y, C, HW, G, g.VC, g.RP, g.P, (const T*)x1, C0, ys, s0, s1, count, eps);
+        else
+            hipLaunchKernelGGL((gn_apply_nhwc<T, false, true>), dim3(g.NB, N), dim3(GN_THREADS), 0, st, (const T*)x, (const T*)gamma,
+                               (const T*)beta, (const float2*)nullptr, (T*)y, C, HW, G, g.VC, g.RP, g.P, (const T*)x1, C0, ys, s0, s1, count, eps);
+        return st_check_launch("group_norm_from_stats");
+    }
+    hipLaunchKernelGGL(gn_cols_finalize, dim3(N * G), dim3(256), 0, st, s0, s1, stats, G, N * G, C / G, count, eps);
     if (silu)
         hipLaunchKernelGGL((gn_apply_nhwc<T, true>), dim3(g.NB, N), dim3(GN_THREADS), 0, st, (const T*)x, (const T*)gamma,
-                           (const T*)beta, stats, (T*)y, C, HW, G, g.VC, g.RP, g.P, (const T*)x1, C0, ys);
+                           (const T*)beta, stats, (T*)y, C, HW, G, g.VC, g.RP, g.P, (const T*)x1, C0, ys, GnSource{}, GnSource{}, 0.0, 0.f);
     else
         hipLaunchKernelGGL((gn_apply_nhwc<T, false>), dim3(g.NB, N), dim3(GN_THREADS), 0, st, (const T*)x, (const T*)gamma,
-                           (const T*)beta, stats, (T*)y, C, HW, G, g.VC, g.RP, g.P, (const T*)x1, C0, ys);
+                           (const T*)beta, stats, (T*)y, C, HW, G, g.VC, g.RP, g.P, (const T*)x1, C0, ys, GnSource{}, GnSource{}, 0.0, 0.f);
     return st_check_launch("group_norm_from_stats");
 }
 
```

Result: slower. 74.72 it/s (-2.2%).
